# beast-dev/beast-mcmc

Measured on NVIDIA H100. Metric: tree log-likelihood evals/sec, higher is better.
Workload: dtype f64

## Files before the change

beast-mcmc_b200/beagle.py:

```python
from __future__ import annotations

import ctypes as C
import os
from typing import Optional, Sequence

import numpy as np

NONE = -1
OPERATION_TUPLE_SIZE = 7
PARTITION_OPERATION_TUPLE_SIZE = 9

_HERE = os.path.dirname(os.path.abspath(__file__))
_LIB = None


class BeagleException(RuntimeError):
    def __init__(self, functionName: str, errCode: int):
        super().__init__(f"BEAGLE function, {functionName}, returned error code {errCode}")
        self.functionName = functionName
        self.errCode = errCode


class BeagleErrorCode:
    NO_ERROR = 0
    GENERAL_ERROR = -1
    OUT_OF_MEMORY_ERROR = -2
    UNIDENTIFIED_EXCEPTION_ERROR = -3
    UNINITIALIZED_INSTANCE_ERROR = -4
    OUT_OF_RANGE_ERROR = -5
    NO_RESOURCE_ERROR = -6
    NO_IMPLEMENTATION_ERROR = -7
    FLOATING_POINT_ERROR = -8


class BeagleFlag:
    PRECISION_SINGLE = 1 << 0
    PRECISION_DOUBLE = 1 << 1
    COMPUTATION_SYNCH = 1 << 2
    COMPUTATION_ASYNCH = 1 << 3
    EIGEN_REAL = 1 << 4
    EIGEN_COMPLEX = 1 << 5
    SCALING_MANUAL = 1 << 6
    SCALING_AUTO = 1 << 7
    SCALING_ALWAYS = 1 << 8
    SCALERS_RAW = 1 << 9
    SCALERS_LOG = 1 << 10
    VECTOR_SSE = 1 << 11
    VECTOR_NONE = 1 << 12
    THREADING_OPENMP = 1 << 13
    THREADING_NONE = 1 << 14
    PROCESSOR_CPU = 1 << 15
    PROCESSOR_GPU = 1 << 16
    SCALING_DYNAMIC = 1 << 19
    FRAMEWORK_CUDA = 1 << 22
    FRAMEWORK_OPENCL = 1 << 23
    FRAMEWORK_CPU = 1 << 27
    PARALLELOPS_STREAMS = 1 << 28
    PARALLELOPS_GRID = 1 << 29
    THREADING_CPP = 1 << 30
    PREORDER_TRANSPOSE_AUTO = 1 << 31
    VECTOR_TENSOR = 1 << 33


class _InstanceDetailsStruct(C.Structure):
    _fields_ = [("resourceNumber", C.c_int), ("resourceName", C.c_char_p), ("implName", C.c_char_p),
                ("implDescription", C.c_char_p), ("flags", C.c_long)]


class _ResourceStruct(C.Structure):
    _fields_ = [("name", C.c_char_p), ("description", C.c_char_p), ("supportFlags", C.c_long),
                ("requiredFlags", C.c_long)]


class _ResourceListStruct(C.Structure):
    _fields_ = [("list", C.POINTER(_ResourceStruct)), ("length", C.c_int)]


class InstanceDetails:
    def __init__(self, resourceNumber=0, flags=0, resourceName="", implementationName=""):
        self.resourceNumber = resourceNumber
        self.flags = flags
        self.resourceName = resourceName
        self.implementationName = implementationName

    def getFlags(self):
        return self.flags

    def getResourceNumber(self):
        return self.resourceNumber


class ResourceDetails:
    def __init__(self, number, name, description, flags):
        self.number, self.name, self.description, self.flags = number, name, description, flags


_I = C.c_int
_IP = C.POINTER(C.c_int)
_DP = C.POINTER(C.c_double)
_L = C.c_long

_SIGNATURES = {
    "beagleGetVersion": ([], C.c_char_p),
    "beagleGetCitation": ([], C.c_char_p),
    "beagleGetResourceList": ([], C.POINTER(_ResourceListStruct)),
    "beagleGetBenchmarkedResourceList": ([_I, _I, _I, _I, _I, _IP, _I, _L, _L, _I, _I, _I, _L], C.c_void_p),
    "beagleCreateInstance": ([_I] * 9 + [_IP, _I, _L, _L, C.POINTER(_InstanceDetailsStruct)], _I),
    "beagleFinalizeInstance": ([_I], _I),
    "beagleFinalize": ([], _I),
    "beagleSetCPUThreadCount": ([_I, _I], _I),
    "beagleSetTipStates": ([_I, _I, _IP], _I),
    "beagleGetTipStates": ([_I, _I, _IP], _I),
    "beagleSetTipPartials": ([_I, _I, _DP], _I),
    "beagleSetPartials": ([_I, _I, _DP], _I),
    "beagleGetPartials": ([_I, _I, _I, _DP], _I),
    "beagleSetEigenDecomposition": ([_I, _I, _DP, _DP, _DP], _I),
    "beagleSetStateFrequencies": ([_I, _I, _DP], _I),
    "beagleSetCategoryWeights": ([_I, _I, _DP], _I),
    "beagleSetCategoryRates": ([_I, _DP], _I),
    "beagleSetCategoryRatesWithIndex": ([_I, _I, _DP], _I),
    "beagleSetPatternWeights": ([_I, _DP], _I),
    "beagleSetPatternPartitions": ([_I, _I, _IP], _I),
    "beagleUpdateTransitionMatrices": ([_I, _I, _IP, _IP, _IP, _DP, _I], _I),
    "beagleUpdateTransitionMatricesWithMultipleModels": ([_I, _IP, _IP, _IP, _IP, _IP, _DP, _I], _I),
    "beagleSetTransitionMatrix": ([_I, _I, _DP, C.c_double], _I),
    "beagleGetTransitionMatrix": ([_I, _I, _DP], _I),
    "beagleSetDifferentialMatrix": ([_I, _I, _DP], _I),
    "beagleConvolveTransitionMatrices": ([_I, _IP, _IP, _IP, _I], _I),
    "beagleAddTransitionMatrices": ([_I, _IP, _IP, _IP, _I], _I),
    "beagleTransposeTransitionMatrices": ([_I, _IP, _IP, _I], _I),
    "beagleUpdatePartials": ([_I, _IP, _I, _I], _I),
    "beagleUpdatePartialsByPartition": ([_I, _IP, _I], _I),
    "beagleWaitForPartials": ([_I, _IP, _I], _I),
    "beagleUpdatePrePartials": ([_I, _IP, _I, _I], _I),
    "beagleUpdatePrePartialsByPartition": ([_I, _IP, _I], _I),
    "beagleAccumulateScaleFactors": ([_I, _IP, _I, _I], _I),
    "beagleAccumulateScaleFactorsByPartition": ([_I, _IP, _I, _I, _I], _I),
    "beagleRemoveScaleFactors": ([_I, _IP, _I, _I], _I),
    "beagleRemoveScaleFactorsByPartition": ([_I, _IP, _I, _I, _I], _I),
    "beagleResetScaleFactors": ([_I, _I], _I),
    "beagleResetScaleFactorsByPartition": ([_I, _I, _I], _I),
    "beagleCopyScaleFactors": ([_I, _I, _I], _I),
    "beagleGetScaleFactors": ([_I, _I, _DP], _I),
    "beagleGetLogScaleFactors": ([_I, _I, _DP], _I),
    "beagleCalculateRootLogLikelihoods": ([_I, _IP, _IP, _IP, _IP, _I, _DP], _I),
    "beagleCalculateRootLogLikelihoodsByPartition": ([_I, _IP, _IP, _IP, _IP, _IP, _I, _I, _DP, _DP], _I),
    "beagleGetSiteLogLikelihoods": ([_I, _DP], _I),
    "beagleCalculateEdgeDerivatives": ([_I, _IP, _IP, _IP, _IP, _I, _DP, _DP, _DP], _I),
    "beagleCalculateCrossProductDerivative": ([_I, _IP, _IP, _IP, _IP, _DP, _I, _DP, _DP], _I),
    "b200SetKernelTiming": ([_I, _I], _I),
    "b200GetKernelTiming": ([_I, _I, _DP, C.POINTER(C.c_long)], _I),
    "b200CompressSitePatterns": ([_I, _I, _I, _IP, _DP, _IP, _IP, _DP, _IP], _I),
    "b200GetSourceHash": ([], C.c_char_p),
    "b200GetFusedLaunches": ([_I], _L),
    "b200RootLogLikelihoodsByPartitionDevice": ([_I, _IP, _IP, _IP, _IP, _IP, _I, C.POINTER(C.c_void_p), C.POINTER(C.c_void_p)], _I),
    "b200SetShardDevices": ([_IP, _I], _I),
    "b200ExchangeConnectLocal": ([_IP, _I], _I),
    "b200ExchangeCreate": ([_I, _I, _I, C.c_void_p], _I),
    "b200ExchangeConnect": ([_I, C.c_void_p], _I),
    "b200HostAlloc": ([_L], C.c_void_p),
    "b200HostFree": ([C.c_void_p], None),
    "b200DebugPlan": ([_I if False else _IP, _I, _I, _I, _I, _I, _I, _I, _IP, _IP, _IP, _IP], _I),
    "b200RootLogLikelihoodDevice": ([_I, _I, _I, _I, _I, C.POINTER(C.c_void_p), C.POINTER(C.c_void_p)], _I),
}


def exported_symbols():
    return list(_SIGNATURES.keys())


def load_library(path: Optional[str] = None):
    global _LIB
    if _LIB is not None and path is None:
        return _LIB
    path = path or os.environ.get("B200_BEAGLE_LIBRARY") or os.path.join(_HERE, "csrc", "libhmsbeagle.so")
    if not os.path.exists(path):
        raise FileNotFoundError(
            f"{path} not found: build it with `python -c 'import __graft_entry__ as g; g.build()'`; "
            "there is no CPU fallback for the product path")
    lib = C.CDLL(path)
    for name, (argtypes, restype) in _SIGNATURES.items():
        fn = getattr(lib, name)
        fn.argtypes = argtypes
        fn.restype = restype
    _LIB = lib
    return lib


def _ip(a):
    if a is None:
        return None
    a = np.ascontiguousarray(a, dtype=np.int32)
    return a, a.ctypes.data_as(_IP)


def _dp(a):
    a = np.ascontiguousarray(a, dtype=np.float64)
    return a, a.ctypes.data_as(_DP)


class Beagle:
    OPERATION_TUPLE_SIZE = OPERATION_TUPLE_SIZE
    PARTITION_OPERATION_TUPLE_SIZE = PARTITION_OPERATION_TUPLE_SIZE
    NONE = NONE


class BeagleJNIImpl(Beagle):

    def __init__(self, tipCount, partialsBufferCount, compactBufferCount, stateCount, patternCount,
                 eigenBufferCount, matrixBufferCount, categoryCount, scaleBufferCount,
                 resourceList: Optional[Sequence[int]], preferenceFlags: int, requirementFlags: int):
        self._lib = load_library()
        det = _InstanceDetailsStruct()
        rl = _ip(resourceList) if resourceList is not None else None
        inst = self._lib.beagleCreateInstance(tipCount, partialsBufferCount, compactBufferCount, stateCount,
                                              patternCount, eigenBufferCount, matrixBufferCount, categoryCount,
                                              scaleBufferCount, rl[1] if rl else None,
                                              len(resourceList) if resourceList is not None else 0,
                                              preferenceFlags, requirementFlags, C.byref(det))
        if inst < 0:
            raise BeagleException("create", inst)
        self.instance = inst
        self.patternCount = patternCount
        self.details = InstanceDetails(det.resourceNumber, det.flags,
                                       (det.resourceName or b"").decode(), (det.implName or b"").decode())

    def _check(self, name, rc):
        if rc != 0:
            raise BeagleException(name, rc)

    def getDetails(self):
        return self.details

    def finalize(self):
        if self.instance >= 0:
            rc = self._lib.beagleFinalizeInstance(self.instance)
            self.instance = -1
            self._check("finalize", rc)

    def setCPUThreadCount(self, threadCount):
        self._check("setCPUThreadCount", self._lib.beagleSetCPUThreadCount(self.instance, threadCount))

    def setPatternWeights(self, patternWeights):
        self._check("setPatternWeights", self._lib.beagleSetPatternWeights(self.instance, _dp(patternWeights)[1]))

    def setPatternPartitions(self, partitionCount, patternPartitions):
        self._check("setPatternPartitions",
                    self._lib.beagleSetPatternPartitions(self.instance, partitionCount, _ip(patternPartitions)[1]))

    def setTipStates(self, tipIndex, states):
        self._check("setTipStates", self._lib.beagleSetTipStates(self.instance, tipIndex, _ip(states)[1]))

    def getTipStates(self, tipIndex, states):
        self._check("getTipStates", self._lib.beagleGetTipStates(self.instance, tipIndex, states.ctypes.data_as(_IP)))

    def setTipPartials(self, tipIndex, partials):
        self._check("setTipPartials", self._lib.beagleSetTipPartials(self.instance, tipIndex, _dp(partials)[1]))

    def setPartials(self, bufferIndex, partials):
        self._check("setPartials", self._lib.beagleSetPartials(self.instance, bufferIndex, _dp(partials)[1]))

    def getPartials(self, bufferIndex, scaleIndex, outPartials):
        assert outPartials.dtype == np.float64 and outPartials.flags.c_contiguous
        self._check("getPartials", self._lib.beagleGetPartials(self.instance, bufferIndex, scaleIndex,
                                                               outPartials.ctypes.data_as(_DP)))

    def getLogScaleFactors(self, scaleIndex, outFactors):
        self._check("getLogScaleFactors", self._lib.beagleGetLogScaleFactors(self.instance, scaleIndex,
                                                                             outFactors.ctypes.data_as(_DP)))

    def getScaleFactors(self, scaleIndex, outFactors):
        self._check("getScaleFactors", self._lib.beagleGetScaleFactors(self.instance, scaleIndex,
                                                                       outFactors.ctypes.data_as(_DP)))

    def setEigenDecomposition(self, eigenIndex, eigenVectors, inverseEigenValues, eigenValues):
        self._check("setEigenDecomposition",
                    self._lib.beagleSetEigenDecomposition(self.instance, eigenIndex, _dp(eigenVectors)[1],
                                                          _dp(inverseEigenValues)[1], _dp(eigenValues)[1]))

    def setStateFrequencies(self, stateFrequenciesIndex, stateFrequencies):
        self._check("setStateFrequencies",
                    self._lib.beagleSetStateFrequencies(self.instance, stateFrequenciesIndex, _dp(stateFrequencies)[1]))

    def setCategoryWeights(self, categoryWeightsIndex, categoryWeights):
        self._check("setCategoryWeights",
                    self._lib.beagleSetCategoryWeights(self.instance, categoryWeightsIndex, _dp(categoryWeights)[1]))

    def setCategoryRates(self, inCategoryRates):
        self._check("setCategoryRates", self._lib.beagleSetCategoryRates(self.instance, _dp(inCategoryRates)[1]))

    def setCategoryRatesWithIndex(self, categoryRatesIndex, inCategoryRates):
        self._check("setCategoryRatesWithIndex",
                    self._lib.beagleSetCategoryRatesWithIndex(self.instance, categoryRatesIndex, _dp(inCategoryRates)[1]))

    def setTransitionMatrix(self, matrixIndex, inMatrix, paddedValue=0.0):
        self._check("setTransitionMatrix",
                    self._lib.beagleSetTransitionMatrix(self.instance, matrixIndex, _dp(inMatrix)[1], paddedValue))

    def getTransitionMatrix(self, matrixIndex, outMatrix):
        self._check("getTransitionMatrix",
                    self._lib.beagleGetTransitionMatrix(self.instance, matrixIndex, outMatrix.ctypes.data_as(_DP)))

    def updateTransitionMatrices(self, eigenIndex, probabilityIndices, firstDerivativeIndices,
                                 secondDerivativeIndices, edgeLengths, count):
        d1 = _ip(firstDerivativeIndices)
        d2 = _ip(secondDerivativeIndices)
        self._check("updateTransitionMatrices",
                    self._lib.beagleUpdateTransitionMatrices(self.instance, eigenIndex, _ip(probabilityIndices)[1],
                                                             d1[1] if d1 else None, d2[1] if d2 else None,
                                                             _dp(edgeLengths)[1], count))

    def updateTransitionMatricesWithMultipleModels(self, eigenIndices, categoryRateIndices, probabilityIndices,
                                                   firstDerivativeIndices, secondDerivativeIndices, edgeLengths, count):
        d1 = _ip(firstDerivativeIndices)
        d2 = _ip(secondDerivativeIndices)
# ... 161 lines not shown
```

beast-mcmc_b200/csrc/api.cu:

```cuda
#include "../../include/libhmsbeagle_b200.h"
#include "engine.h"
#include "multi.h"

#include <algorithm>
#include <atomic>
#include <chrono>
#include <cmath>
#include <cstdio>
#include <cstdlib>
#include <cstring>
#include <string>
#include <unordered_map>

using namespace b200;

namespace {

std::mutex gMutex;
std::vector<Instance*> gInstances;

const long kSupportedFlags =
    BEAGLE_FLAG_PRECISION_DOUBLE | BEAGLE_FLAG_PRECISION_SINGLE | BEAGLE_FLAG_COMPUTATION_SYNCH | BEAGLE_FLAG_EIGEN_REAL |
    BEAGLE_FLAG_EIGEN_COMPLEX | BEAGLE_FLAG_SCALING_MANUAL | BEAGLE_FLAG_SCALING_DYNAMIC |
    BEAGLE_FLAG_SCALERS_RAW | BEAGLE_FLAG_SCALERS_LOG | BEAGLE_FLAG_VECTOR_NONE | BEAGLE_FLAG_THREADING_NONE |
// ... 206 lines not shown
        plan.order.resize(n);
        for (int k = 0; k < n; ++k) plan.order[k] = k;
        plan.subs.assign(1, Sub{0, n, 0, 0});
        plan.phaseStart = {0, 1};
    };
    if (!allowReorder || n < 2) { single(); return; }
    std::vector<int> writer(nBuffers, -1);
    for (int k = 0; k < n; ++k) {
        if (writer[ops[k].dest] >= 0) { single(); return; }
        writer[ops[k].dest] = k;
    }
    std::vector<int> ch0(n, -1), ch1(n, -1), parent(n, -1);
    for (int k = 0; k < n; ++k) {
        const int a = writer[ops[k].c1], b = writer[ops[k].c2];
        if (a >= 0) { if (a >= k || parent[a] >= 0) { single(); return; } ch0[k] = a; parent[a] = k; }
        if (b >= 0 && ops[k].c2 != ops[k].c1) { if (b >= k || parent[b] >= 0) { single(); return; } ch1[k] = b; parent[b] = k; }
        if (ops[k].dest == ops[k].c1 || ops[k].dest == ops[k].c2) { single(); return; }
    }
    std::vector<char> alive(n, 1);
    std::vector<int> size(n), need(n);
    std::vector<std::pair<int, int>> stack;
    plan.order.clear(); plan.order.reserve(n);
    plan.subs.clear(); plan.phaseStart.assign(1, 0);
    int remaining = n;
    while (remaining > 0) {
        const int T = fixedT > 0 ? fixedT : (remaining <= smallRemainder ? remaining : std::max(minT, (remaining + wantSubs - 1) / wantSubs));
        for (int k = 0; k < n; ++k) {
            if (!alive[k]) continue;
            const int a = (ch0[k] >= 0 && alive[ch0[k]]) ? ch0[k] : -1;
            const int b = (ch1[k] >= 0 && alive[ch1[k]]) ? ch1[k] : -1;
            size[k] = 1 + (a >= 0 ? size[a] : 0) + (b >= 0 ? size[b] : 0);
            int na = a >= 0 ? need[a] : 0, nb = b >= 0 ? need[b] : 0;
            if (na < nb) std::swap(na, nb);
            need[k] = std::max(1, std::max(na, nb + (nb > 0 ? 1 : 0)));
        }
        for (int r = 0; r < n; ++r) {
            if (!alive[r] || size[r] > T) continue;
            if (parent[r] >= 0 && size[parent[r]] <= T) continue;
            const int begin = (int)plan.order.size();
            stack.push_back({r, 0});
            while (!stack.empty()) {
                auto [k, stageNo] = stack.back();
                stack.pop_back();
                if (stageNo == 1) { plan.order.push_back(k); continue; }
                stack.push_back({k, 1});
                const int a = (ch0[k] >= 0 && alive[ch0[k]]) ? ch0[k] : -1;
                const int b = (ch1[k] >= 0 && alive[ch1[k]]) ? ch1[k] : -1;
                const int na = a >= 0 ? need[a] : -1, nb = b >= 0 ? need[b] : -1;
                if (na >= nb) { if (b >= 0) stack.push_back({b, 0}); if (a >= 0) stack.push_back({a, 0}); }
                else          { if (a >= 0) stack.push_back({a, 0}); if (b >= 0) stack.push_back({b, 0}); }
            }
            plan.subs.push_back(Sub{begin, (int)plan.order.size(), 0, 0});
        }
        for (int q = plan.subs[plan.phaseStart.back()].begin; q < (int)plan.order.size(); ++q) alive[plan.order[q]] = 0;
        std::stable_sort(plan.subs.begin() + plan.phaseStart.back(), plan.subs.end(),
                         [](const Sub& a, const Sub& b) { return (a.end - a.begin) > (b.end - b.begin); });
        remaining = n - (int)plan.order.size();
        plan.phaseStart.push_back((int)plan.subs.size());
    }
}

void planLevels(const std::vector<HostOp>& ops, int nBuffers, Plan& plan) {
    const int n = (int)ops.size();
    std::vector<int> writer(nBuffers, -1), level(n, 0);
    bool hazard = false;
    for (int k = 0; k < n; ++k) { if (writer[ops[k].dest] >= 0) hazard = true; writer[ops[k].dest] = k; }
    int maxLevel = 0;
    for (int k = 0; k < n && !hazard; ++k) {
        for (int src : {ops[k].c1, ops[k].c2}) {
            const int w = writer[src];
            if (w < 0) continue;
            if (w >= k) { hazard = true; break; }
            level[k] = std::max(level[k], level[w] + 1);
        }
        maxLevel = std::max(maxLevel, level[k]);
    }
    plan.order.resize(n);
    for (int k = 0; k < n; ++k) plan.order[k] = k;
    plan.subs.clear();
    if (hazard) { plan.subs.assign(1, Sub{0, n, 0, 0}); plan.phaseStart = {0, 1}; return; }
    std::stable_sort(plan.order.begin(), plan.order.end(), [&](int a, int b) { return level[a] < level[b]; });
    plan.phaseStart.assign(1, 0);
    for (int pos = 0; pos < n; ++pos) {
        if (pos > 0 && level[plan.order[pos]] != level[plan.order[pos - 1]]) plan.phaseStart.push_back((int)plan.subs.size());
        plan.subs.push_back(Sub{pos, pos + 1, 0, 0});
    }
    plan.phaseStart.push_back((int)plan.subs.size());
}

void planPreorderPhases(const std::vector<HostOp>& ops, int nBuffers, int fixedT, int wantSubs, int minT,
                        int smallRemainder, Plan& plan) {
    const int n = (int)ops.size();
    std::vector<int> writer(nBuffers, -1), parent(n, -1);
    bool ok = n >= 2;
    for (int k = 0; k < n && ok; ++k) { ok = writer[ops[k].dest] < 0; writer[ops[k].dest] = k; }
    for (int k = 0; k < n && ok; ++k) {
        const int a = writer[ops[k].c1];
        ok = writer[ops[k].c2] < 0 && (a < 0 || a < k) && ops[k].dest != ops[k].c1 && ops[k].dest != ops[k].c2;
        parent[k] = a;
    }
    if (!ok) { planLevels(ops, nBuffers, plan); return; }
    std::vector<std::vector<int>> kids(n);
    for (int k = 0; k < n; ++k) if (parent[k] >= 0) kids[parent[k]].push_back(k);
    std::vector<char> alive(n, 1);
    std::vector<int> size(n), stack;
    std::vector<std::vector<int>> phases;
    int remaining = n;
    while (remaining > 0) {
        const int T = fixedT > 0 ? fixedT : (remaining <= smallRemainder ? remaining : std::max(minT, (remaining + wantSubs - 1) / wantSubs));
        for (int k = n - 1; k >= 0; --k) {
            if (!alive[k]) continue;
            size[k] = 1;
            for (int c : kids[k]) if (alive[c]) size[k] += size[c];
        }
        std::vector<int> roots;
        for (int r = 0; r < n; ++r)
            if (alive[r] && size[r] <= T && !(parent[r] >= 0 && alive[parent[r]] && size[parent[r]] <= T)) roots.push_back(r);
        for (int r : roots) {
            stack.assign(1, r);
            while (!stack.empty()) {
                const int k = stack.back(); stack.pop_back();
                if (!alive[k]) continue;
                alive[k] = 0; --remaining;
                for (int c : kids[k]) if (alive[c]) stack.push_back(c);
            }
        }
        phases.push_back(std::move(roots));
    }
    std::vector<int> phaseOf(n, -1), rootOf(n, -1);
    for (int ph = 0; ph < (int)phases.size(); ++ph)
        for (int r : phases[ph]) { phaseOf[r] = ph; rootOf[r] = r; }
    for (int k = 0; k < n; ++k)
        if (rootOf[k] < 0) { rootOf[k] = rootOf[parent[k]]; phaseOf[k] = phaseOf[parent[k]]; }
    plan.order.clear(); plan.order.reserve(n);
    plan.subs.clear(); plan.phaseStart.assign(1, 0);
    for (int ph = (int)phases.size() - 1; ph >= 0; --ph) {
        for (int r : phases[ph]) {
            const int begin = (int)plan.order.size();
            stack.assign(1, r);
            while (!stack.empty()) {
                const int k = stack.back(); stack.pop_back();
                plan.order.push_back(k);
                for (int q = (int)kids[k].size() - 1; q >= 0; --q)
                    if (rootOf[kids[k][q]] == r) stack.push_back(kids[k][q]);
            }
            plan.subs.push_back(Sub{begin, (int)plan.order.size(), 0, 0});
        }
        std::stable_sort(plan.subs.begin() + plan.phaseStart.back(), plan.subs.end(),
                         [](const Sub& a, const Sub& b) { return (a.end - a.begin) > (b.end - b.begin); });
        plan.phaseStart.push_back((int)plan.subs.size());
    }
}

cudaError_t launchPlan(Instance* in, const void* dOps, const void* dSubs, const std::vector<int>& phaseStart,
                       const std::vector<int>& phaseDepth, bool fourPath, int maxWindow, bool preOrder, int eigenSlot = -1,
                       bool aligned = false, const void* dSnap = nullptr, int nSnap = 0, const void* dVirtTips = nullptr) {
    const bool virt = dVirtTips != nullptr;
    cudaError_t e = cudaSuccess;
    if (nSnap > 0) {
        TimedScope ts(in, T_PARTIALS);
        e = launchCherrySnapshot(in, static_cast<const int4*>(dSnap), nSnap);
    }
    for (size_t ph = 0; ph + 1 < phaseStart.size() && e == cudaSuccess; ++ph) {
        const int s0 = phaseStart[ph], s1 = phaseStart[ph + 1];
        if (s1 <= s0) continue;
        TimedScope ts(in, T_PARTIALS);
        if (fourPath && eigenSlot >= 0 && !preOrder && (ph >= phaseDepth.size() || phaseDepth[ph] == 0)) {
            e = launchWalk4E(in, static_cast<const Op4*>(dOps), static_cast<const int4*>(dSubs) + s0, s1 - s0, maxWindow,
                             aligned, in->hEigen.data() + (size_t)eigenSlot * 36, static_cast<const int4*>(dVirtTips));
            continue;
        }
        if (virt) return cudaErrorInvalidValue;
        e = fourPath ? launchWalk4(in, static_cast<const Op4*>(dOps), static_cast<const int4*>(dSubs) + s0, s1 - s0,
                                   ph < phaseDepth.size() ? phaseDepth[ph] : 0, maxWindow, preOrder)
                     : launchWalkGeneric(in, static_cast<const DevOp*>(dOps), static_cast<const int4*>(dSubs) + s0, s1 - s0,
                                         maxWindow, preOrder);
    }
    return e;
}

cudaError_t accumulateInList(Instance* in, const std::vector<CumGroup>& groups) {
    for (const CumGroup& g : groups) {
        int* dIdx = static_cast<int*>(stage(in, g.indices.data(), sizeof(int) * g.indices.size()));
        if (dIdx == nullptr) return cudaErrorMemoryAllocation;
        cudaError_t e = launchScaleAccumulate(in, dIdx, (int)g.indices.size(), in->dScale + (size_t)g.cum * in->Ppad, 1.0,
                                              g.pBegin, g.pEnd);
        if (e != cudaSuccess) return e;
        in->scaleIsLog[g.cum] = 1;
    }
    return cudaSuccess;
}

void noteScaleWrites(Instance* in, const std::vector<HostOp>& hops) {
    for (const HostOp& o : hops) if (o.sw >= 0) in->scaleIsLog[o.sw] = in->logScalers ? 1 : 0;
}


cudaError_t storeCherries(Instance* in, const int* bufs, int count) {
    if (in->cherryTip1.empty()) return cudaSuccess;
    std::vector<int4> items;
    for (int k = 0; k < count; ++k) {
        const int b = bufs[k];
        if (!validRange(b, in->nBuffers) || in->cherryTip1[b] < 0 || in->cherryStored[b]) continue;
        items.push_back(make_int4(in->slotOf[b], b, in->cherryTip1[b], in->cherryTip2[b]));
        in->cherryStored[b] = 1;
    }
    if (items.empty()) return cudaSuccess;
    const int4* dItems = static_cast<const int4*>(stage(in, items.data(), sizeof(int4) * items.size()));
    cudaError_t e = cudaErrorMemoryAllocation;
    if (dItems != nullptr) {
        TimedScope ts(in, T_PARTIALS);
        e = launchCherryStore(in, dItems, (int)items.size());
    }
    if (e != cudaSuccess) for (const int4& it : items) in->cherryStored[it.y] = 0;
    return e;
}

cudaError_t storeExternal(Instance* in, const std::vector<CherryRef>& external) {
    std::vector<int> bufs;
    for (const CherryRef& x : external) if (x.tip1 < 0) bufs.push_back(x.buf);
    return storeCherries(in, bufs.data(), (int)bufs.size());
}

cudaError_t settleCherriesOf(Instance* in, int t) {
    std::vector<int> deps;
    for (int b = 0; b < (int)in->cherryTip1.size(); ++b)
        if (in->cherryTip1[b] >= 0 && (in->cherryTip1[b] == t || in->cherryTip2[b] == t)) deps.push_back(b);
    const cudaError_t e = storeCherries(in, deps.data(), (int)deps.size());
    if (e == cudaSuccess) for (int b : deps) in->cherryTip1[b] = -1;
    return e;
}

void noteCherryWrites(Instance* in, const std::vector<HostOp>& hops, const std::vector<CherryRef>& cherries) {
    if (in->cherryTip1.empty()) return;
    for (const HostOp& o : hops) in->cherryTip1[o.dest] = -1;
    for (const CherryRef& c : cherries) {
        in->cherryTip1[c.buf] = c.tip1; in->cherryTip2[c.buf] = c.tip2; in->cherryStored[c.buf] = 0;
    }
}

int prepareOps(Instance* in, const std::vector<HostOp>& hops, bool byPartition) {
    for (const HostOp& o : hops) {
        if (!validRange(o.dest, in->nBuffers) || !validRange(o.c1, in->nBuffers) ||
            !validRange(o.c2, in->nBuffers) || !validRange(o.m1, in->nMatrices) ||
            !validRange(o.m2, in->nMatrices))
            return BEAGLE_ERROR_OUT_OF_RANGE;
        if (o.sw != BEAGLE_OP_NONE && !validRange(o.sw, in->nScale)) return BEAGLE_ERROR_OUT_OF_RANGE;
        if (o.sr != BEAGLE_OP_NONE && !validRange(o.sr, in->nScale)) return BEAGLE_ERROR_OUT_OF_RANGE;
        if (o.cum != BEAGLE_OP_NONE && !validRange(o.cum, in->nScale)) return BEAGLE_ERROR_OUT_OF_RANGE;
        if (byPartition && !validRange(o.part, in->partitionCount)) return BEAGLE_ERROR_OUT_OF_RANGE;
    }
    {
        std::vector<char> written(in->nBuffers, 0);
        for (const HostOp& o : hops) written[o.dest] = 1;
        auto holdsData = [&](int b) { return written[b] || in->partials[b] != nullptr || in->states32[b] != nullptr; };
        for (const HostOp& o : hops) {
            if (!holdsData(o.c1) || !holdsData(o.c2)) return BEAGLE_ERROR_OUT_OF_RANGE;
            if (o.kind == 1 && !written[o.c1] && in->states32[o.c1] != nullptr) return BEAGLE_ERROR_OUT_OF_RANGE;
        }
    }
    for (const HostOp& o : hops) {
        if (ensurePartials(in, o.dest) == nullptr) return BEAGLE_ERROR_OUT_OF_MEMORY;
        if (in->states32[o.dest] != nullptr) in->bufferEpoch++;
        in->states8[o.dest] = nullptr;
        in->states32[o.dest] = nullptr;
    }
    return BEAGLE_SUCCESS;
}

int eigenFormSlot(const Instance* in, const std::vector<HostOp>& hops) {
    if (!in->eigenWalk || in->matCP == 0 || in->walkVariant != 0 || hops.empty() || hops[0].kind == 1) return -1;
    const int E = in->matEigen[hops[0].m1];
    if (E < 0 || !in->eigenReal[E]) return -1;
    const unsigned gen = in->eigenGen[E];
    for (const HostOp& o : hops)
        if (in->matEigen[o.m1] != E || in->matEigen[o.m2] != E || in->matEigenGen[o.m1] != gen || in->matEigenGen[o.m2] != gen)
            return -1;
    return E;
}

int planAndLaunch(Instance* in, const std::vector<HostOp>& hops, bool byPartition) {
    const int n = (int)hops.size();
    if (n == 0) return BEAGLE_SUCCESS;
    static_assert(sizeof(HostOp) == 10 * sizeof(int), "HostOp is compared bytewise");
    if (in->planCacheSize > 0) {
        for (CachedPlan& cp : in->planCache) {
            if (cp.dBlock == nullptr || cp.n != n || cp.byPartition != byPartition || cp.epoch != in->bufferEpoch ||
                memcmp(cp.key.data(), hops.data(), sizeof(HostOp) * (size_t)n) != 0)
                continue;
            const int eigenSlot = cp.fourPath ? eigenFormSlot(in, hops) : -1;
            bool stale = cp.readsVirtual && eigenSlot < 0;
            for (const CherryRef& x : cp.external)
                stale = stale || (x.tip1 >= 0 && (in->cherryTip1[x.buf] != x.tip1 || in->cherryTip2[x.buf] != x.tip2));
            if (stale) { cp.dropGraph(); cp.n = -1; continue; }
            CUDA_OK(storeExternal(in, cp.external));
            cp.lastUse = ++in->planClock;
            cp.hits++;
            const unsigned eigenGenNow = eigenSlot >= 0 ? in->eigenGen[eigenSlot] : 0u;
            const void* dSnap = static_cast<char*>(cp.dBlock) + cp.snapOffset;
            const int nSnap = (int)cp.cherries.size();
            const void* dTips = cp.readsVirtual ? static_cast<char*>(cp.dBlock) + cp.tipsOffset : nullptr;
            if (cp.graphExec != nullptr && (cp.graphEigen != eigenSlot || cp.graphEigenGen != eigenGenNow)) {
                if (cp.graphAllEigen && eigenSlot >= 0 && cp.graphEigen == eigenSlot &&
                    updateWalk4EGraph(cp.graphExec, cp.graphKernelNodes, in->hEigen.data() + (size_t)eigenSlot * 36) == cudaSuccess) {
                    cp.graphEigenGen = eigenGenNow;
                } else {
                    cudaGetLastError();
                    cp.dropGraph();
                    cp.hits = 1;
                    if (++cp.graphInvalidations >= 4) cp.graphFailed = true;
                }
            }
            int launches = nSnap > 0;
            for (size_t ph = 0; ph + 1 < cp.phaseStart.size(); ++ph) launches += cp.phaseStart[ph + 1] > cp.phaseStart[ph];
            if (in->useGraphs && launches >= 2 && cp.cumGroups.empty()) {
                if (cp.graphExec == nullptr && !cp.graphFailed && cp.hits >= 2 && !in->timing &&
                    cudaStreamBeginCapture(in->stream, cudaStreamCaptureModeThreadLocal) == cudaSuccess) {
                    const cudaError_t e1 = launchPlan(in, cp.dBlock, static_cast<char*>(cp.dBlock) + cp.subsOffset, cp.phaseStart,
                                                      cp.phaseDepth, cp.fourPath, cp.maxWindow, cp.preOrder, eigenSlot,
                                                      !cp.byPartition, dSnap, nSnap, dTips);
                    cp.graphEigen = eigenSlot;
                    cp.graphEigenGen = eigenGenNow;
                    cudaGraph_t g = nullptr;
                    const cudaError_t e2 = cudaStreamEndCapture(in->stream, &g);
                    if (e1 != cudaSuccess || e2 != cudaSuccess || g == nullptr ||
                        cudaGraphInstantiate(&cp.graphExec, g, 0) != cudaSuccess) {
                        cp.graphExec = nullptr;
                        cp.graphFailed = true;
                        if (g) cudaGraphDestroy(g);
                    } else {
                        cp.graph = g;
                        cp.graphKernelNodes.clear();
                        cp.graphAllEigen = cp.fourPath && eigenSlot >= 0 && !cp.preOrder;
                        for (int dpt : cp.phaseDepth) cp.graphAllEigen = cp.graphAllEigen && dpt == 0;
                        size_t nn = 0;
                        if (cudaGraphGetNodes(g, nullptr, &nn) == cudaSuccess && nn > 0) {
                            std::vector<cudaGraphNode_t> nodes(nn);
                            cudaGraphNodeType ty;
                            if (cudaGraphGetNodes(g, nodes.data(), &nn) == cudaSuccess)
                                for (size_t q = 0; q < nn; ++q)
                                    if (cudaGraphNodeGetType(nodes[q], &ty) == cudaSuccess && ty == cudaGraphNodeTypeKernel)
                                        cp.graphKernelNodes.push_back(nodes[q]);
                        }
                        if (cp.graphKernelNodes.empty()) cp.graphAllEigen = false;
                    }
                    if (getenv("B200_BEAGLE_DEBUG"))
                        fprintf(stderr, "[b200-beagle] graph %s: %d launches\n", cp.graphExec ? "captured" : "capture failed",
                                launches);
                    cudaGetLastError();
                }
                if (cp.graphExec != nullptr) {
                    TimedScope ts(in, T_PARTIALS, launches);
                    CUDA_OK(cudaGraphLaunch(cp.graphExec, in->stream));
                    noteScaleWrites(in, hops);
                    noteCherryWrites(in, hops, cp.cherries);
                    return BEAGLE_SUCCESS;
                }
            }
            CUDA_OK(launchPlan(in, cp.dBlock, static_cast<char*>(cp.dBlock) + cp.subsOffset, cp.phaseStart, cp.phaseDepth,
                               cp.fourPath, cp.maxWindow, cp.preOrder, eigenSlot, !cp.byPartition, dSnap, nSnap,
                               dTips));
            CUDA_OK(accumulateInList(in, cp.cumGroups));
            noteScaleWrites(in, hops);
            noteCherryWrites(in, hops, cp.cherries);
            return BEAGLE_SUCCESS;
        }
    }
    {
        const int rcPrepare = prepareOps(in, hops, byPartition);
        if (rcPrepare != BEAGLE_SUCCESS) return rcPrepare;
    }
    const bool fourState = in->matCP > 0;
    const bool preOrder = hops[0].kind == 1;
    const int eigenSlot = fourState ? eigenFormSlot(in, hops) : -1;
    std::vector<char> written(in->nBuffers, 0);
    std::vector<int> firstWrite(in->nBuffers, n);
    for (int k = n - 1; k >= 0; --k) { written[hops[k].dest] = 1; firstWrite[hops[k].dest] = k; }
    std::vector<CherryRef> cherries;
    std::vector<int4> snap;
    std::vector<HostOp> kept;
    bool readsVirtual = false;
    if (!in->cherryTip1.empty() && !byPartition && !preOrder && eigenSlot >= 0 && !in->stackTail) {
        std::vector<int> writes(in->nBuffers, 0), firstRead(in->nBuffers, n);
        for (int k = 0; k < n; ++k) {
            writes[hops[k].dest]++;
            firstRead[hops[k].c1] = std::min(firstRead[hops[k].c1], k);
            firstRead[hops[k].c2] = std::min(firstRead[hops[k].c2], k);
        }
        for (int k = 0; k < n; ++k) {
            const HostOp& o = hops[k];
            if (in->states8[o.c1] != nullptr && in->states8[o.c2] != nullptr && o.sw == BEAGLE_OP_NONE &&
                o.sr == BEAGLE_OP_NONE && o.cum == BEAGLE_OP_NONE && writes[o.dest] == 1 && firstRead[o.dest] > k) {
                cherries.push_back(CherryRef{o.dest, o.c1, o.c2});
                snap.push_back(make_int4(o.dest, o.m1, o.m2, 0));
            } else {
                kept.push_back(o);
            }
        }
        if (kept.empty()) { cherries.clear(); snap.clear(); }
        readsVirtual = !cherries.empty();
        for (const HostOp& o : hops)
            for (int c : {o.c1, o.c2})
                readsVirtual = readsVirtual || (!written[c] && in->states32[c] == nullptr && in->cherryTip1[c] >= 0);
    }
    Plan plan;
    int maxWindow = in->Ppad;
    const int patsPerWarp = !fourState ? 16 : (in->walkVariant == 2 ? 8 * in->tensorR : (32 / in->matCP) * in->walkR);
    const int warpsPerSM = fourState ? 32 : 12;
    auto wantSubsFor = [&](int window) {
        const int warpsPerSub = std::max(1, (window + patsPerWarp - 1) / patsPerWarp);
        const int over = in->phaseOversub > 0 ? in->phaseOversub : (warpsPerSub >= 32 ? 1 : 2);
        return std::max(1, over * ((in->smCount * warpsPerSM + warpsPerSub - 1) / warpsPerSub));
    };
    if (!byPartition && !preOrder) {
        planPhases(cherries.empty() ? hops : kept, in->nBuffers, in->reorder != 0, in->phaseT, wantSubsFor(in->Ppad),
                   in->phaseTmin, in->phaseSmall, plan);
        bool served = true;
        for (size_t ph = 0; readsVirtual && ph + 1 < plan.phaseStart.size(); ++ph) {
            const int nSubs = plan.phaseStart[ph + 1] - plan.phaseStart[ph];
            served = served && (nSubs == 0 || walk4pServes(in, nSubs, in->Ppad));
        }
        if (!served) {
            readsVirtual = false;
            if (!cherries.empty()) {
                cherries.clear(); snap.clear(); kept.clear();
                planPhases(hops, in->nBuffers, in->reorder != 0, in->phaseT, wantSubsFor(in->Ppad), in->phaseTmin,
                           in->phaseSmall, plan);
            }
        }
        for (Sub& sb : plan.subs) { sb.pBase = 0; sb.pLimit = in->Ppad; }
    }
    const std::vector<HostOp>& L = cherries.empty() ? hops : kept;
    const int nL = (int)L.size();
    std::vector<int> vt1(readsVirtual ? in->nBuffers : 0, -1), vt2(readsVirtual ? in->nBuffers : 0, -1);
    for (const CherryRef& c : cherries) { vt1[c.buf] = c.tip1; vt2[c.buf] = c.tip2; }
    std::vector<CherryRef> external;
    {
        std::vector<char> seen(in->nBuffers, 0);
        for (int k = 0; k < n; ++k)
            for (int c : {hops[k].c1, hops[k].c2}) {
                if (firstWrite[c] < k || in->states32[c] != nullptr || seen[c]) continue;
                seen[c] = 1;
                const bool virt = readsVirtual && !written[c] && in->cherryTip1[c] >= 0;
                external.push_back(CherryRef{c, virt ? in->cherryTip1[c] : -1, virt ? in->cherryTip2[c] : -1});
                if (virt) { vt1[c] = in->cherryTip1[c]; vt2[c] = in->cherryTip2[c]; }
            }
    }
    CUDA_OK(storeExternal(in, external));
    {
        if (!byPartition) {
            if (preOrder) {
                if (in->prePhases) planPreorderPhases(hops, in->nBuffers, in->phaseT, wantSubsFor(in->Ppad), in->phaseTmin, in->phaseSmall, plan);
                else planLevels(hops, in->nBuffers, plan);
                for (Sub& sb : plan.subs) { sb.pBase = 0; sb.pLimit = in->Ppad; }
            }
        } else {
            std::vector<std::vector<int>> members(in->partitionCount);
            for (int k = 0; k < n; ++k) members[hops[k].part].push_back(k);
            std::vector<Plan> plans;
            std::vector<int> base;
            maxWindow = 1;
            for (int part = 0; part < in->partitionCount; ++part) {
                if (members[part].empty()) continue;
                std::vector<HostOp> sub(members[part].size());
                for (size_t q = 0; q < sub.size(); ++q) sub[q] = hops[members[part][q]];
                Plan pl;
                const int window = in->partEnd[part] - in->partBegin[part];
                if (sub[0].kind == 1 && in->prePhases) planPreorderPhases(sub, in->nBuffers, in->phaseT, wantSubsFor(std::max(1, window)), in->phaseTmin, in->phaseSmall, pl);
                else if (sub[0].kind == 1) planLevels(sub, in->nBuffers, pl);
                else planPhases(sub, in->nBuffers, in->reorder != 0, in->phaseT, wantSubsFor(std::max(1, window)), in->phaseTmin, in->phaseSmall, pl);
                base.push_back((int)plan.order.size());
                for (int idx : pl.order) plan.order.push_back(members[part][idx]);
                for (Sub& sb : pl.subs) {
                    sb.begin += base.back(); sb.end += base.back();
                    sb.pBase = in->partBegin[part]; sb.pLimit = in->partEnd[part];
                }
                maxWindow = std::max(maxWindow, window);
                plans.push_back(std::move(pl));
            }
            plan.phaseStart.assign(1, 0);
            for (size_t ph = 0;; ++ph) {
                bool any = false;
                for (const Plan& pl : plans) {
                    if (ph + 1 >= pl.phaseStart.size()) continue;
                    any = true;
                    for (int q = pl.phaseStart[ph]; q < pl.phaseStart[ph + 1]; ++q) plan.subs.push_back(pl.subs[q]);
                }
                if (!any) break;
                plan.phaseStart.push_back((int)plan.subs.size());
            }
        }
    }
    const std::vector<int>& order = plan.order;

    const bool stackEverywhere = fourState && in->walkVariant == 1 && !preOrder;
    const bool stackThin = fourState && in->walkVariant == 0 && in->stackTail && !preOrder;
    const int maxDepth = (stackEverywhere || stackThin) ? in->stackDepthMax : 0;
    const int nPhases = (int)plan.phaseStart.size() - 1;
    std::vector<char> subStack(plan.subs.size(), 0);
    std::vector<int> phaseDepth(std::max(nPhases, 1), 0), phaseOfSub(plan.subs.size(), 0);
    if (maxDepth > 0) {
        const int patsPerWarpS = (32 / in->matCP) * in->walkR;
        for (int ph = 0; ph < nPhases; ++ph) {
            long warps = 0;
            for (int q = plan.phaseStart[ph]; q < plan.phaseStart[ph + 1]; ++q) {
                warps += (plan.subs[q].pLimit - plan.subs[q].pBase + patsPerWarpS - 1) / patsPerWarpS;
                phaseOfSub[q] = ph;
            }
            const bool thin = warps < (long)in->smCount * 8;
            for (int q = plan.phaseStart[ph]; q < plan.phaseStart[ph + 1]; ++q) subStack[q] = stackEverywhere || thin;
        }
    }
    std::vector<int> lastReadOfProd(maxDepth > 0 ? nL : 0, -1);
    std::vector<int> subOfPos(nL, 0);
    for (int sIdx = 0; sIdx < (int)plan.subs.size(); ++sIdx)
        for (int q = plan.subs[sIdx].begin; q < plan.subs[sIdx].end; ++q) subOfPos[q] = sIdx;
    if (maxDepth > 0) {
        std::vector<int> lastRead(in->nBuffers, -1);
        for (size_t sIdx = 0; sIdx < plan.subs.size(); ++sIdx) {
            if (!subStack[sIdx]) continue;
            const Sub& sb = plan.subs[sIdx];
            for (int pos = sb.end - 1; pos >= sb.begin; --pos) {
                const HostOp& o = L[order[pos]];
                lastReadOfProd[pos] = lastRead[o.dest];
                lastRead[o.dest] = -1;
                if (lastRead[o.c1] < 0) lastRead[o.c1] = pos;
                if (lastRead[o.c2] < 0) lastRead[o.c2] = pos;
            }
            for (int pos = sb.begin; pos < sb.end; ++pos) {
                const HostOp& o = L[order[pos]];
                lastRead[o.dest] = lastRead[o.c1] = lastRead[o.c2] = -1;
            }
        }
    }
    std::vector<int> slotOf(maxDepth > 0 ? in->nBuffers : 0, -1), slotFreeAt(maxDepth > 0 ? in->nBuffers : 0, -1);
    std::vector<int> freeSlots;
    int depthUsed = 0, depthThisSub = 0, curSub = -1;

    const bool fourPath = in->matCP > 0;
    std::vector<CumGroup> cumGroups;
    std::vector<DevOp> dops(fourPath ? 0 : nL);
    std::vector<Op4> ops4(fourPath ? nL : 0);
    std::vector<int4> virtTips(readsVirtual ? nL : 0);
    for (int pos = 0; pos < nL; ++pos) {
        const HostOp& o = L[order[pos]];
        const bool t1 = in->states32[o.c1] != nullptr;
        const bool t2 = in->states32[o.c2] != nullptr;
        int srcSlot1 = -1, srcSlot2 = -1, dstSlot = -1;
        if (maxDepth > 0 && subOfPos[pos] != curSub) {
            curSub = subOfPos[pos];
            freeSlots.clear();
            depthThisSub = 0;
        }
        if (maxDepth > 0 && subStack[subOfPos[pos]]) {
            auto take = [&](int buf, bool isTip) -> int {
                if (isTip) return -1;
                const int slot = slotOf[buf];
                if (slot >= 0 && slotFreeAt[buf] == pos) { freeSlots.push_back(slot); slotOf[buf] = -1; }
                return slot;
            };
            srcSlot1 = take(o.c1, t1);
            srcSlot2 = (o.c2 == o.c1) ? srcSlot1 : take(o.c2, t2);
            if (slotOf[o.dest] >= 0) { freeSlots.push_back(slotOf[o.dest]); slotOf[o.dest] = -1; }
            if (lastReadOfProd[pos] > pos) {
                int slot = -1;
                if (!freeSlots.empty()) { slot = freeSlots.back(); freeSlots.pop_back(); }
                else if (depthThisSub < maxDepth) {
                    slot = depthThisSub++;
                    depthUsed = std::max(depthUsed, depthThisSub);
                    phaseDepth[phaseOfSub[subOfPos[pos]]] = std::max(phaseDepth[phaseOfSub[subOfPos[pos]]], depthThisSub);
                }
                if (slot >= 0) { slotOf[o.dest] = slot; slotFreeAt[o.dest] = lastReadOfProd[pos]; dstSlot = slot; }
            }
        }
        const int pBegin = byPartition ? in->partBegin[o.part] : 0;
        const int pEnd = byPartition ? in->partEnd[o.part] : in->P;
        if (o.cum >= 0 && o.sw >= 0) {
            CumGroup* grp = nullptr;
            for (CumGroup& g : cumGroups) if (g.cum == o.cum && g.pBegin == pBegin && g.pEnd == pEnd) { grp = &g; break; }
            if (grp == nullptr) { cumGroups.push_back(CumGroup{o.cum, pBegin, pEnd, {}}); grp = &cumGroups.back(); }
            grp->indices.push_back(o.sw);
        }
        const int cum = -1;
        if (fourPath) {
            Op4& d = ops4[pos];
            const bool v1 = readsVirtual && !t1 && vt1[o.c1] >= 0, v2 = readsVirtual && !t2 && vt1[o.c2] >= 0;
            d.dest = in->slotOf[o.dest];
            d.c1 = t1 ? -(o.c1 + 1) : v1 ? o.c1 : in->slotOf[o.c1];
            d.c2 = t2 ? -(o.c2 + 1) : v2 ? o.c2 : in->slotOf[o.c2];
            d.m1 = o.m1; d.m2 = o.m2; d.sw = o.sw; d.sr = o.sr; d.cum = cum;
            d.pBegin = pBegin; d.pEnd = pEnd;
            d.slots = (unsigned)(srcSlot1 & 0xFF) | ((unsigned)(srcSlot2 & 0xFF) << 8) | ((unsigned)(dstSlot & 0xFF) << 16);
            d.pad_ = o.kind | (v1 ? 4 : 0) | (v2 ? 8 : 0);
            d.pfA = d.pfB = 0; d.pfM1 = d.pfM2 = -1;
            if (readsVirtual)
                virtTips[pos] = make_int4(v1 ? vt1[o.c1] : 0, v1 ? vt2[o.c1] : 0, v2 ? vt1[o.c2] : 0, v2 ? vt2[o.c2] : 0);
            if (in->forward && !(maxDepth > 0 && subStack[subOfPos[pos]]) && pos > plan.subs[subOfPos[pos]].begin) {
                const Op4& pv = ops4[pos - 1];
                if (pv.pBegin == d.pBegin && pv.pEnd == d.pEnd) {
                    if (!t1 && !v1 && d.c1 == pv.dest) d.pad_ |= 2;
                    else if (!preOrder && !t2 && !v2 && d.c2 == pv.dest) {
                        std::swap(d.c1, d.c2); std::swap(d.m1, d.m2);
                        if (readsVirtual) { int4& t = virtTips[pos]; t = make_int4(t.z, t.w, t.x, t.y); }
                        d.pad_ = (d.pad_ & ~12) | (v1 ? 8 : 0) | 2;
                    }
                }
            }
        } else {
            DevOp& d = dops[pos];
            memset(&d, 0, sizeof d);
            d.dest = reinterpret_cast<double*>(in->partials[o.dest]);
            d.c1 = t1 ? nullptr : reinterpret_cast<const double*>(in->partials[o.c1]);
            d.c2 = t2 ? nullptr : reinterpret_cast<const double*>(in->partials[o.c2]);
            d.s1 = t1 ? (const void*)in->states32[o.c1] : nullptr;
            d.s2 = t2 ? (const void*)in->states32[o.c2] : nullptr;
            d.m1 = in->dMat + (size_t)o.m1 * in->matStride;
            d.m2 = in->dMat + (size_t)o.m2 * in->matStride;
            d.scaleWrite = o.sw >= 0 ? in->dScale + (size_t)o.sw * in->Ppad : nullptr;
            d.scaleRead = o.sr >= 0 ? in->dScale + (size_t)o.sr * in->Ppad : nullptr;
            d.cumScale = cum >= 0 ? in->dScale + (size_t)cum * in->Ppad : nullptr;
            d.pBegin = pBegin; d.pEnd = pEnd;
            d.srcSlot1 = d.srcSlot2 = d.dstSlot = -1;
            d.pad_ = o.kind;
            if (in->forward && !preOrder && pos > plan.subs[subOfPos[pos]].begin) {
                const DevOp& pv = dops[pos - 1];
                if (pv.pBegin == d.pBegin && pv.pEnd == d.pEnd) {
                    if (d.c1 != nullptr && d.c1 == pv.dest) d.pad_ |= 2;
                    else if (d.c2 != nullptr && d.c2 == pv.dest) {
                        std::swap(d.c1, d.c2); std::swap(d.s1, d.s2); std::swap(d.m1, d.m2); d.pad_ |= 2;
                    }
                }
            }
        }
    }
    if (fourPath && in->lookahead && (!preOrder || in->lookaheadPre)) {
        std::vector<char> thick(plan.subs.size(), 0);
        const long perSub = (maxWindow + (32 / in->matCP) * in->walkR - 1) / ((32 / in->matCP) * in->walkR);
        for (int ph = 0; ph < nPhases; ++ph) {
            const bool t = (long)(plan.phaseStart[ph + 1] - plan.phaseStart[ph]) * perSub >= (long)in->smCount * 8;
            for (int q = plan.phaseStart[ph]; q < plan.phaseStart[ph + 1]; ++q) thick[q] = t;
        }
        for (size_t sIdx = 0; sIdx < plan.subs.size(); ++sIdx) {
            if ((maxDepth > 0 && subStack[sIdx]) || (!thick[sIdx] && in->lookahead < 2)) continue;
            for (int pos = plan.subs[sIdx].begin; pos + 1 < plan.subs[sIdx].end; ++pos) {
                Op4& d = ops4[pos];
                const Op4& nx = ops4[pos + 1];
                auto enc = [&](int child, bool fromRegisters, bool virt) -> int {
                    if (fromRegisters || virt) return 0;
                    if (child < 0) return ((-child - 1) << 1) | 1;
                    return child == d.dest ? 0 : ((child + 1) << 1);
                };
                d.pfA = enc(nx.c1, (nx.pad_ & 2) != 0, (nx.pad_ & 4) != 0);
                d.pfB = enc(nx.c2, false, (nx.pad_ & 8) != 0);
                if (d.pfA == 0) { d.pfA = d.pfB; d.pfB = 0; }
                d.pfM1 = nx.m1; d.pfM2 = nx.m2;
            }
        }
    }
    if (fourPath && getenv("B200_BEAGLE_DEBUG")) {
        int fwd = 0, internal = 0;
        for (const Op4& d : ops4) { fwd += (d.pad_ & 2) != 0; internal += (d.c1 >= 0) + (d.c2 >= 0); }
        fprintf(stderr, "[b200-beagle] plan: %d ops (%zu virtual cherries), %zu subtrees, %d phases, %d internal children, "
                "%d forwarded in registers\n", nL, cherries.size(), plan.subs.size(), nPhases, internal, fwd);
    }
    const size_t opBytes = (fourPath ? sizeof(Op4) : sizeof(DevOp)) * (size_t)nL;
    const size_t subBytes = sizeof(Sub) * plan.subs.size();
    const size_t snapBytes = sizeof(int4) * snap.size();
    const size_t subsOffset = (opBytes + 255) & ~size_t(255);
    const size_t snapOffset = subsOffset + ((subBytes + 255) & ~size_t(255));
    const size_t tipsBytes = sizeof(int4) * virtTips.size();
    const size_t tipsOffset = snapOffset + ((snapBytes + 255) & ~size_t(255));
    const size_t blockBytes = tipsOffset + tipsBytes;
    std::vector<char> hBlock(blockBytes, 0);
    memcpy(hBlock.data(), fourPath ? (const void*)ops4.data() : (const void*)dops.data(), opBytes);
    memcpy(hBlock.data() + subsOffset, plan.subs.data(), subBytes);
    if (snapBytes) memcpy(hBlock.data() + snapOffset, snap.data(), snapBytes);
    if (tipsBytes) memcpy(hBlock.data() + tipsOffset, virtTips.data(), tipsBytes);
    void* dOps = stage(in, hBlock.data(), blockBytes);
    void* tmp = nullptr;
    if (dOps == nullptr) {
        CUDA_OK(cudaMalloc(&tmp, blockBytes));
        dOps = tmp;
        cudaError_t ce = cudaMemcpyAsync(dOps, hBlock.data(), blockBytes, cudaMemcpyHostToDevice, in->stream);
        if (ce == cudaSuccess) ce = cudaStreamSynchronize(in->stream);
        if (ce != cudaSuccess) { cudaFree(tmp); CUDA_OK(ce); }
    }
    void* dSubs = static_cast<char*>(dOps) + subsOffset;
    std::vector<int> depths(plan.phaseStart.size(), 0);
    for (size_t ph = 0; ph + 1 < plan.phaseStart.size(); ++ph) depths[ph] = (maxDepth > 0 && ph < phaseDepth.size()) ? phaseDepth[ph] : 0;
    cudaError_t e = launchPlan(in, dOps, dSubs, plan.phaseStart, depths, fourPath, maxWindow, preOrder, eigenSlot, !byPartition,
                               static_cast<char*>(dOps) + snapOffset, (int)snap.size(),
                               readsVirtual ? static_cast<char*>(dOps) + tipsOffset : nullptr);
    if (e == cudaSuccess) e = accumulateInList(in, cumGroups);
    noteScaleWrites(in, hops);
    if (e == cudaSuccess) noteCherryWrites(in, hops, cherries);
    if (e == cudaSuccess && tmp == nullptr && in->planCacheSize > 0) {
        if ((int)in->planCache.size() < in->planCacheSize) in->planCache.emplace_back();
        CachedPlan* slot = nullptr;
        for (CachedPlan& cp : in->planCache) {
            if (cp.dBlock == nullptr || cp.n < 0) { slot = &cp; break; }
            if (slot == nullptr || cp.lastUse < slot->lastUse) slot = &cp;
        }
        slot->dropGraph();
        slot->hits = 0;
        slot->graphFailed = false;
        slot->graphInvalidations = 0;
        if (slot->capacity < blockBytes) {
            if (slot->dBlock) cudaFree(slot->dBlock);
            slot->dBlock = nullptr; slot->capacity = 0;
            if (cudaMalloc(&slot->dBlock, blockBytes) == cudaSuccess) slot->capacity = blockBytes; else cudaGetLastError();
        }
        if (slot->dBlock != nullptr &&
            cudaMemcpyAsync(slot->dBlock, dOps, blockBytes, cudaMemcpyDeviceToDevice, in->stream) == cudaSuccess) {
            slot->key = hops; slot->n = n; slot->byPartition = byPartition; slot->epoch = in->bufferEpoch;
            slot->subsOffset = subsOffset; slot->snapOffset = snapOffset; slot->tipsOffset = tipsOffset;
            slot->cherries = cherries; slot->external = external; slot->readsVirtual = readsVirtual;
            slot->phaseStart = plan.phaseStart; slot->phaseDepth = depths;
            slot->fourPath = fourPath; slot->maxWindow = maxWindow; slot->preOrder = preOrder;
            slot->lastUse = ++in->planClock;
            slot->cumGroups = cumGroups;
            slot->graphFailed = !cumGroups.empty();
        } else if (slot->dBlock != nullptr) {
            slot->n = -1;
        }
    }
    if (tmp != nullptr) { cudaStreamSynchronize(in->stream); cudaFree(tmp); }
    CUDA_OK(e);
    return BEAGLE_SUCCESS;
}

}

namespace b200 {
Instance* instanceById(int id) { return getInstance(id); }
}

extern "C" {

#ifndef B200_SOURCE_HASH
#define B200_SOURCE_HASH "unhashed"
#endif
const char* beagleGetVersion(void) { return "4.0.1-b200+" B200_SOURCE_HASH; }
const char* b200GetSourceHash(void) { return B200_SOURCE_HASH; }

const char* beagleGetCitation(void) {
    return "H100-native tree-likelihood engine exposing the BEAGLE API.\n"
           "API after: Ayres et al. (2019) BEAGLE 3. Syst Biol 68:1052-1061.";
}

BeagleResourceList* beagleGetResourceList(void) {
    std::call_once(gResourceOnce, buildResources);
    return &gResourceList;
}

BeagleBenchmarkedResourceList* beagleGetBenchmarkedResourceList(
    int tipCount, int compactBufferCount, int stateCount, int patternCount, int categoryCount, int* resourceList,
    int resourceCount, long preferenceFlags, long requirementFlags, int eigenModelCount, int partitionCount,
    int calculateDerivatives, long benchmarkFlags);

int beagleCreateInstance(int tipCount, int partialsBufferCount, int compactBufferCount, int stateCount,
                         int patternCount, int eigenBufferCount, int matrixBufferCount, int categoryCount,
                         int scaleBufferCount, int* resourceList, int resourceCount, long preferenceFlags,
                         long requirementFlags, BeagleInstanceDetails* returnInfo) {
    if (tipCount < 0 || partialsBufferCount < 0 || compactBufferCount < 0 || stateCount < 2 ||
        patternCount < 1 || eigenBufferCount < 0 || matrixBufferCount < 0 || categoryCount < 1 ||
        scaleBufferCount < 0 || stateCount > 255)
        return BEAGLE_ERROR_OUT_OF_RANGE;
    if (requirementFlags & ~kSupportedFlags) return BEAGLE_ERROR_NO_RESOURCE;
    const bool singleFits = stateCount <= 4 && categoryCount <= 8;
    if (requirementFlags & BEAGLE_FLAG_PRECISION_SINGLE) {
        if (!singleFits || (requirementFlags & BEAGLE_FLAG_PRECISION_DOUBLE)) return BEAGLE_ERROR_NO_RESOURCE;
    }
    const bool single = singleFits && ((requirementFlags & BEAGLE_FLAG_PRECISION_SINGLE) ||
                                       ((preferenceFlags & BEAGLE_FLAG_PRECISION_SINGLE) &&
                                        !((preferenceFlags | requirementFlags) & BEAGLE_FLAG_PRECISION_DOUBLE)));
    BeagleResourceList* rl = beagleGetResourceList();
    int resource = -1;
    if (resourceList == nullptr || resourceCount <= 0) {
        if (rl->length > 1) resource = 1;
    } else {
        for (int k = 0; k < resourceCount; ++k)
            if (resourceList[k] >= 1 && resourceList[k] < rl->length) { resource = resourceList[k]; break; }
    }
    if (resource < 1) return BEAGLE_ERROR_NO_RESOURCE;

    if (resource == gShardResource) {
        Instance* parent = new Instance();
        parent->resource = resource;
        parent->device = gShardDevices[0];
        parent->P = patternCount; parent->S = stateCount; parent->C = categoryCount; parent->tipCount = tipCount;
        const int g = (int)gShardDevices.size();
        const int rc = shardedCreate(parent, g, gShardDevices.data(), tipCount, partialsBufferCount, compactBufferCount,
                                     stateCount, patternCount, eigenBufferCount, matrixBufferCount, categoryCount,
                                     scaleBufferCount, preferenceFlags, requirementFlags, returnInfo);
        if (rc != BEAGLE_SUCCESS) { delete parent; return rc; }
        if (returnInfo != nullptr) {
            returnInfo->resourceNumber = resource;
            returnInfo->resourceName = rl->list[resource].name;
            parent->flags = returnInfo->flags;
        }
        std::lock_guard<std::mutex> lock(gMutex);
        int id = -1;
        for (size_t k = 0; k < gInstances.size(); ++k) if (gInstances[k] == nullptr) { id = (int)k; break; }
        if (id < 0) { gInstances.push_back(nullptr); id = (int)gInstances.size() - 1; }
        gInstances[id] = parent;
        parent->id = id;
        return id;
    }

    Instance* in = new Instance();
    in->device = resource - 1;
    in->resource = resource;
    if (cudaSetDevice(in->device) != cudaSuccess) { delete in; return BEAGLE_ERROR_NO_RESOURCE; }
    in->tipCount = tipCount; in->nPartials = partialsBufferCount; in->nCompact = compactBufferCount;
    in->S = stateCount; in->P = patternCount; in->nEigen = eigenBufferCount; in->nMatrices = matrixBufferCount;
    in->C = categoryCount; in->nScale = scaleBufferCount;
    in->Sp = stateCount <= 4 ? 4 : ((stateCount + 7) / 8) * 8;
    in->Ppad = ((patternCount + 31) / 32) * 32;
    in->nBuffers = partialsBufferCount + compactBufferCount;
    in->nSets = std::max(1, eigenBufferCount);
    in->single = single;
    in->complexEigen = (requirementFlags | preferenceFlags) & BEAGLE_FLAG_EIGEN_COMPLEX;
    in->logScalers = (requirementFlags | preferenceFlags) & BEAGLE_FLAG_SCALERS_LOG;
    in->flags = (single ? BEAGLE_FLAG_PRECISION_SINGLE : BEAGLE_FLAG_PRECISION_DOUBLE) | BEAGLE_FLAG_COMPUTATION_SYNCH |
                BEAGLE_FLAG_SCALING_MANUAL |
                BEAGLE_FLAG_VECTOR_NONE | BEAGLE_FLAG_THREADING_NONE | BEAGLE_FLAG_PROCESSOR_GPU |
                BEAGLE_FLAG_FRAMEWORK_CUDA | BEAGLE_FLAG_PARALLELOPS_GRID |
                (in->complexEigen ? BEAGLE_FLAG_EIGEN_COMPLEX : BEAGLE_FLAG_EIGEN_REAL) |
                (in->logScalers ? BEAGLE_FLAG_SCALERS_LOG : BEAGLE_FLAG_SCALERS_RAW);
    if ((requirementFlags | preferenceFlags) & BEAGLE_FLAG_PREORDER_TRANSPOSE_AUTO) in->flags |= BEAGLE_FLAG_PREORDER_TRANSPOSE_AUTO;
    if ((requirementFlags | preferenceFlags) & BEAGLE_FLAG_SCALING_DYNAMIC) {
        in->flags &= ~BEAGLE_FLAG_SCALING_MANUAL;
        in->flags |= BEAGLE_FLAG_SCALING_DYNAMIC;
    }
    in->partialsElems = (size_t)in->C * in->Ppad * in->Sp;
    if (in->Sp == 4 && in->C <= 32) {
        int cp = 1;
        while (cp < in->C) cp <<= 1;
        in->matCP = cp;
        in->matStride = (size_t)16 * cp + 52 * (size_t)in->C;
        in->matStride = (in->matStride + 3) & ~size_t(3);
    } else {
        in->matCP = 0;
        in->matStride = (size_t)in->C * in->Sp * (in->Sp + 2 * (size_t)(in->Sp + 4));
    }
    in->slotOf.assign(in->nBuffers, -1);
    in->partials.assign(in->nBuffers, nullptr);
    in->states8.assign(in->nBuffers, nullptr);
    in->states32.assign(in->nBuffers, nullptr);
    in->scaleIsLog.assign(std::max(1, in->nScale), in->logScalers ? 1 : 0);
    in->matEigen.assign(std::max(1, in->nMatrices), -1);
    in->matEigenGen.assign(std::max(1, in->nMatrices), 0u);
    in->eigenGen.assign(std::max(1, in->nEigen), 0u);
    in->eigenReal.assign(std::max(1, in->nEigen), 0);
    in->hEigen.assign((size_t)std::max(1, in->nEigen) * 36, 0.0);
    in->eigenWalk = envInt("B200_EIGEN_WALK", 1);
    in->tipMode = envInt("B200_TIP_MODE", 3);
    in->thinTipMode = envInt("B200_THIN_TIP_MODE", in->tipMode);
    in->virtualCherries = envInt("B200_VIRTUAL_CHERRIES", 1);
    in->walkBlock = 128;
    in->walkVariant = envInt("B200_WALK_VARIANT", 0);
    in->reorder = envInt("B200_REORDER", 1);
    in->forward = envInt("B200_FORWARD", 1);
    in->lookahead = envInt("B200_LOOKAHEAD", 1);
    in->useGraphs = envInt("B200_GRAPHS", 1);
    in->prePhases = envInt("B200_PRE_PHASES", 1);
    in->lookaheadPre = envInt("B200_LOOKAHEAD_PRE", 1);
    in->planCacheSize = std::max(0, std::min(16, envInt("B200_PLAN_CACHE", 4)));
    in->planCache.reserve(16);
    in->thinR1 = envInt("B200_THIN_R1", 1);
    in->stackTail = envInt("B200_STACK_TAIL", 0);
    in->phaseT = envInt("B200_PHASE_T", 0);
    in->phaseTmin = std::max(1, envInt("B200_PHASE_TMIN", 4));
    in->phaseSmall = envInt("B200_PHASE_SMALL", 24);
    in->phaseOversub = std::max(0, envInt("B200_PHASE_OVERSUB", 0));
    in->walkMinBlocks = envInt("B200_WALK_MINB", 4);
    in->walkMinBlocksSet = getenv("B200_WALK_MINB") != nullptr;
    in->tensorR = envInt("B200_TENSOR_R", 2) >= 4 ? 4 : 2;
    in->genericMma = envInt("B200_GENERIC_MMA", 1);
    in->mmaWarps = envInt("B200_MMA_WARPS", 4) == 8 ? 8 : 4;
    cudaDeviceProp prop;
    bool ok = cudaGetDeviceProperties(&prop, in->device) == cudaSuccess;
    if (ok) { in->smCount = prop.multiProcessorCount; in->maxSmemOptin = prop.sharedMemPerBlockOptin; }
    in->walkR = envInt("B200_WALK_R", 4);
    if (in->walkR != 1 && in->walkR != 2 && in->walkR != 4 && in->walkR != 8) in->walkR = 4;
    if (getenv("B200_WALK_R") == nullptr && in->matCP > 0) {
        const int G = 32 / in->matCP;
        while (in->walkR > 1 && (in->Ppad + G * in->walkR - 1) / (G * in->walkR) < in->smCount) in->walkR >>= 1;
    }
    in->stackDepthMax = std::min(64, std::max(0, envInt("B200_STACK_DEPTH", 12)));
    if (single) { in->walkVariant = 0; in->stackTail = 0; }

    ok = ok && cudaStreamCreateWithFlags(&in->stream, cudaStreamNonBlocking) == cudaSuccess;
    const size_t eigenStride = 2 * (size_t)in->S * in->S + 2 * in->S;
    const size_t matElems = (size_t)in->nMatrices * in->matStride;
    const int rootBlocks = (in->Ppad + 255) / 256;
    in->stageSize = size_t(8) << 20;
    auto alloc = [&](auto** p, size_t elems) {
        if (!ok) return;
        using T = std::remove_pointer_t<std::remove_pointer_t<decltype(p)>>;
        size_t bytes = std::max<size_t>(elems, 1) * sizeof(T);
        ok = cudaMalloc(reinterpret_cast<void**>(p), bytes) == cudaSuccess &&
             cudaMemsetAsync(*p, 0, bytes, in->stream) == cudaSuccess;
    };
    alloc(&in->dEigen, std::max(1, in->nEigen) * eigenStride);
    alloc(&in->dMat, matElems);
    if (in->matCP > 0) alloc(&in->dEvec, (size_t)in->nMatrices * in->matCP * 4);
    if (in->matCP > 0 && in->matCP <= 8 && in->virtualCherries) {
        alloc(&in->dRecipe, (size_t)in->nBuffers * 32 * in->matCP);
        in->cherryTip1.assign(in->nBuffers, -1);
        in->cherryTip2.assign(in->nBuffers, -1);
        in->cherryStored.assign(in->nBuffers, 0);
    }
    if (in->matCP > 0 && in->matCP <= 8) {
        alloc(&in->dIncSums, (size_t)in->Ppad / 4 + 8);
        alloc(&in->dIncCounter, 4);
        in->fuseSmall = envInt("B200_FUSE", 1);
        if (ok && in->fuseSmall) {
            if (cudaHostAlloc(reinterpret_cast<void**>(&in->hMapped), 64, cudaHostAllocMapped) == cudaSuccess &&
                cudaHostGetDevicePointer(reinterpret_cast<void**>(&in->dMapped), in->hMapped, 0) == cudaSuccess) {
                memset(in->hMapped, 0, 64);
            } else {
                cudaGetLastError();
                if (in->hMapped) cudaFreeHost(in->hMapped);
                in->hMapped = nullptr;
            }
        }
    }
    alloc(&in->dRates, (size_t)in->nSets * in->C);
    alloc(&in->dWeights, (size_t)in->nSets * in->C);
    alloc(&in->dFreqs, (size_t)in->nSets * in->Sp);
    alloc(&in->dScale, (size_t)in->nScale * in->Ppad);
    alloc(&in->dPatternWeights, in->Ppad);
    alloc(&in->dPatternPartitions, in->Ppad);
    alloc(&in->dSite, in->Ppad);
    alloc(&in->dBlockSums, rootBlocks);
    alloc(&in->dOut, 1024);
    alloc(&in->dCounter, 4);
    alloc(&in->dStage, in->stageSize);
    alloc(&in->states8Base, (size_t)std::max(1, in->tipCount) * in->Ppad);
    alloc(&in->states32Base, (size_t)std::max(1, in->tipCount) * in->Ppad);
    if (ok) {
        int want[2] = {in->nPartials, std::max(1, in->nPartials - std::min(in->nCompact, in->tipCount))};
        for (int attempt = 0; attempt < 2 && in->partialsBase == nullptr; ++attempt) {
            size_t bytes = (size_t)want[attempt] * in->partialsElems * in->elemBytes();
            if (cudaMalloc(reinterpret_cast<void**>(&in->partialsBase), bytes) == cudaSuccess) in->nSlots = want[attempt];
            else { cudaGetLastError(); in->partialsBase = nullptr; }
        }
        if (in->partialsBase == nullptr) { destroyInstance(in); return BEAGLE_ERROR_OUT_OF_MEMORY; }
    }
    ok = ok && cudaMallocHost(reinterpret_cast<void**>(&in->hStage), in->stageSize) == cudaSuccess;
    ok = ok && cudaMallocHost(reinterpret_cast<void**>(&in->hOut), 1024 * sizeof(double)) == cudaSuccess;
    if (ok) {
        in->hRates.assign((size_t)in->nSets * in->C, 1.0);
        in->hWeights.assign((size_t)in->nSets * in->C, 0.0);
        in->hFreqs.assign((size_t)in->nSets * 4, 0.0);
        std::vector<double> ones((size_t)std::max(in->nSets * in->C, in->Ppad), 1.0);
        ok = cudaMemcpyAsync(in->dRates, ones.data(), sizeof(double) * in->nSets * in->C, cudaMemcpyHostToDevice,
                             in->stream) == cudaSuccess;
        std::vector<double> w(in->Ppad, 0.0);
        std::fill(w.begin(), w.begin() + in->P, 1.0);
        ok = ok && cudaMemcpyAsync(in->dPatternWeights, w.data(), sizeof(double) * in->Ppad, cudaMemcpyHostToDevice,
                                   in->stream) == cudaSuccess;
        ok = ok && cudaStreamSynchronize(in->stream) == cudaSuccess;
    }
    if (!ok) {
        cudaError_t e = cudaGetLastError();
        destroyInstance(in);
        return e == cudaErrorMemoryAllocation ? BEAGLE_ERROR_OUT_OF_MEMORY : BEAGLE_ERROR_GENERAL;
    }
    in->partitionCount = 1;
    in->partBegin.assign(1, 0);
    in->partEnd.assign(1, in->P);
    {
        std::lock_guard<std::mutex> lock(gMutex);
        int id = -1;
        for (size_t k = 0; k < gInstances.size(); ++k) if (gInstances[k] == nullptr) { id = (int)k; break; }
        if (id < 0) { gInstances.push_back(nullptr); id = (int)gInstances.size() - 1; }
        gInstances[id] = in;
        in->id = id;
    }
    if (returnInfo != nullptr) {
        returnInfo->resourceNumber = resource;
        returnInfo->resourceName = rl->list[resource].name;
        returnInfo->implName = single ? gImplNameSingle : gImplName;
        returnInfo->implDescription = gImplDesc;
        returnInfo->flags = in->flags;
    }
    return in->id;
}

int beagleFinalizeInstance(int instance) {
    Instance* in = nullptr;
    {
        std::lock_guard<std::mutex> lock(gMutex);
        if (instance < 0 || instance >= (int)gInstances.size() || gInstances[instance] == nullptr)
            return BEAGLE_ERROR_UNINITIALIZED_INSTANCE;
        in = gInstances[instance];
        gInstances[instance] = nullptr;
    }
    destroyInstance(in);
    return BEAGLE_SUCCESS;
}

int beagleFinalize(void) {
    std::vector<Instance*> all;
    {
        std::lock_guard<std::mutex> lock(gMutex);
        all.swap(gInstances);
    }
    for (Instance* in : all) if (in) destroyInstance(in);
    return BEAGLE_SUCCESS;
}

int beagleSetCPUThreadCount(int instance, int) {
    SH(instance, BEAGLE_SUCCESS);
// ... 762 lines not shown
                                                 const int* categoryWeightsIndices,
                                                 const int* stateFrequenciesIndices,
                                                 const int* cumulativeScaleIndices, const int* partitionIndices,
                                                 int partitionCount, int count,
                                                 double* outSumLogLikelihoodByPartition, double* outSumLogLikelihood) {
    SH(instance, BEAGLE_ERROR_NO_IMPLEMENTATION);
    GET_INSTANCE(in, instance);
    if (count != 1) return BEAGLE_ERROR_NO_IMPLEMENTATION;
    int rc = rootByPartitionLaunch(in, bufferIndices, categoryWeightsIndices, stateFrequenciesIndices,
                                   cumulativeScaleIndices, partitionIndices, partitionCount);
    if (rc != BEAGLE_SUCCESS) return rc;
    const int extra = in->exchangeOn ? 2 : 0;
    CUDA_OK(cudaMemcpyAsync(in->hOut, in->dOut, sizeof(double) * (partitionCount + extra), cudaMemcpyDeviceToHost, in->stream));
    CUDA_OK(cudaStreamSynchronize(in->stream));
    double total = 0.0;
    for (int k = 0; k < partitionCount; ++k) { outSumLogLikelihoodByPartition[k] = in->hOut[k]; total += in->hOut[k]; }
    if (in->exchangeOn) total = in->hOut[partitionCount];
    *outSumLogLikelihood = total;
    return std::isnan(total) ? BEAGLE_ERROR_FLOATING_POINT : BEAGLE_SUCCESS;
}

int beagleGetSiteLogLikelihoods(int instance, double* outLogLikelihoods) {
    SH(instance, shGetPerPattern(sh, outLogLikelihoods, [&](int c, double* o) { return beagleGetSiteLogLikelihoods(c, o); }));
    GET_INSTANCE(in, instance);
    CUDA_OK(cudaMemcpyAsync(outLogLikelihoods, in->dSite, sizeof(double) * in->P, cudaMemcpyDeviceToHost, in->stream));
    CUDA_OK(cudaStreamSynchronize(in->stream));
    return BEAGLE_SUCCESS;
}

static cudaError_t ensureScratch(Instance* in, size_t doubles) {
    if (doubles <= in->scratchDoubles) return cudaSuccess;
    cudaError_t e = cudaStreamSynchronize(in->stream);
    if (e != cudaSuccess) return e;
    cudaFree(in->dScratch);
    in->dScratch = nullptr;
    in->scratchDoubles = 0;
    e = cudaMalloc(reinterpret_cast<void**>(&in->dScratch), doubles * sizeof(double));
    if (e == cudaSuccess) in->scratchDoubles = doubles;
    return e;
}

int beagleCalculateEdgeDerivatives(int instance, const int* postBufferIndices, const int* preBufferIndices,
                                   const int* derivativeMatrixIndices, const int* categoryWeightsIndices, int count,
                                   double* outDerivatives, double* outSumDerivatives, double* outSumSquaredDerivatives) {
    SH(instance, shEdgeDerivatives(sh, postBufferIndices, preBufferIndices, derivativeMatrixIndices, categoryWeightsIndices, count, outDerivatives, outSumDerivatives, outSumSquaredDerivatives));
    GET_INSTANCE(in, instance);
    if (count <= 0) return BEAGLE_SUCCESS;
    if (!validRange(categoryWeightsIndices[0], in->nSets)) return BEAGLE_ERROR_OUT_OF_RANGE;
    std::vector<EdgeRefT<void>> edges(count);
    for (int e = 0; e < count; ++e) {
        const int po = postBufferIndices[e], pr = preBufferIndices[e], dm = derivativeMatrixIndices[e];
        if (!validRange(po, in->nBuffers) || !validRange(pr, in->nBuffers) || !validRange(dm, in->nMatrices) ||
            in->partials[pr] == nullptr || (in->partials[po] == nullptr && in->states32[po] == nullptr))
            return BEAGLE_ERROR_OUT_OF_RANGE;
        edges[e].post = in->states32[po] != nullptr ? nullptr : in->partials[po];
        edges[e].states = in->states32[po];
        edges[e].pre = in->partials[pr];
        edges[e].D = in->dMat + (size_t)dm * in->matStride;
        edges[e].len = 0.0;
    }
    CUDA_OK(storeCherries(in, postBufferIndices, count));
    const size_t perEdge = outDerivatives != nullptr ? (size_t)in->P : 0;
    const size_t edgeDoubles = ((size_t)count * sizeof(EdgeRefT<void>) + 7) / 8;
    const size_t results = (size_t)count * (2 + perEdge);
    const size_t partials = edgeDerivativeWorkspace(in, count);
    CUDA_OK(ensureScratch(in, edgeDoubles + results + partials));
    EdgeRefT<void>* dEdges = reinterpret_cast<EdgeRefT<void>*>(in->dScratch);
    double* dOut = in->dScratch + edgeDoubles;
    CUDA_OK(cudaMemcpyAsync(dEdges, edges.data(), sizeof(EdgeRefT<void>) * count, cudaMemcpyHostToDevice, in->stream));
    {
        TimedScope ts(in, T_ROOT);
        CUDA_OK(launchEdgeDerivatives(in, dEdges, count, in->dWeights + (size_t)categoryWeightsIndices[0] * in->C,
                                      perEdge ? dOut + 2 * (size_t)count : nullptr, dOut, dOut + count,
                                      partials ? dOut + results : nullptr));
    }
    std::vector<double> host(results);
    CUDA_OK(cudaMemcpyAsync(host.data(), dOut, sizeof(double) * results, cudaMemcpyDeviceToHost, in->stream));
    CUDA_OK(cudaStreamSynchronize(in->stream));
    for (int k = 0; k < count; ++k) {
        if (outSumDerivatives) outSumDerivatives[k] = host[k];
        if (outSumSquaredDerivatives) outSumSquaredDerivatives[k] = host[count + k];
    }
    if (outDerivatives) memcpy(outDerivatives, host.data() + 2 * (size_t)count, sizeof(double) * (size_t)count * in->P);
    return BEAGLE_SUCCESS;
}

int beagleCalculateCrossProductDerivative(int instance, const int* postBufferIndices, const int* preBufferIndices,
                                          const int* categoryRatesIndices, const int* categoryWeightsIndices,
                                          const double* edgeLengths, int count, double* outSumDerivatives,
                                          double* outSumSquaredDerivatives) {
    SH(instance, shCrossProducts(sh, postBufferIndices, preBufferIndices, categoryRatesIndices, categoryWeightsIndices, edgeLengths, count, outSumDerivatives, outSumSquaredDerivatives));
    GET_INSTANCE(in, instance);
    if (outSumSquaredDerivatives != nullptr) return BEAGLE_ERROR_NO_IMPLEMENTATION;
    if (count <= 0) return BEAGLE_SUCCESS;
    if (outSumDerivatives == nullptr || edgeLengths == nullptr) return BEAGLE_ERROR_OUT_OF_RANGE;
    if (!validRange(categoryRatesIndices[0], in->nSets) || !validRange(categoryWeightsIndices[0], in->nSets))
        return BEAGLE_ERROR_OUT_OF_RANGE;
    const size_t n = (size_t)in->S * in->S;
    const size_t edgeDoubles = ((size_t)count * sizeof(EdgeRefT<void>) + 7) / 8;
    const size_t need = edgeDoubles + ((size_t)crossProductBlocks(in, count) + 1) * n;
    CUDA_OK(ensureScratch(in, need));
    std::vector<EdgeRefT<void>> edges(count);
    for (int e = 0; e < count; ++e) {
        const int po = postBufferIndices[e], pr = preBufferIndices[e];
        if (!validRange(po, in->nBuffers) || !validRange(pr, in->nBuffers) || in->partials[pr] == nullptr ||
            (in->partials[po] == nullptr && in->states32[po] == nullptr))
            return BEAGLE_ERROR_OUT_OF_RANGE;
        edges[e].post = in->states32[po] != nullptr ? nullptr : in->partials[po];
        edges[e].states = in->states32[po];
        edges[e].pre = in->partials[pr];
        edges[e].D = nullptr;
        edges[e].len = edgeLengths[e];
    }
    CUDA_OK(storeCherries(in, postBufferIndices, count));
    EdgeRefT<void>* dEdges = reinterpret_cast<EdgeRefT<void>*>(in->dScratch);
    double* work = in->dScratch + edgeDoubles;
    CUDA_OK(cudaMemcpyAsync(dEdges, edges.data(), sizeof(EdgeRefT<void>) * count, cudaMemcpyHostToDevice, in->stream));
    {
        TimedScope ts(in, T_ROOT);
        CUDA_OK(launchCrossProducts(in, dEdges, count, in->dRates + (size_t)categoryRatesIndices[0] * in->C,
                                    in->dWeights + (size_t)categoryWeightsIndices[0] * in->C, work));
    }
    std::vector<double> host(n);
    CUDA_OK(cudaMemcpyAsync(host.data(), work + (size_t)crossProductBlocks(in, count) * n, sizeof(double) * n,
                            cudaMemcpyDeviceToHost, in->stream));
    CUDA_OK(cudaStreamSynchronize(in->stream));
    for (size_t q = 0; q < n; ++q) outSumDerivatives[q] += host[q];
    return BEAGLE_SUCCESS;
}

int b200DebugPlan(const int* operations, int operationCount, int bufferCount, int fixedT, int wantSubs, int minT,
                  int smallRemainder, int preOrder, int* outOrder, int* outSubs, int* outPhaseStart, int* outCounts) {
    if (operationCount < 0 || bufferCount <= 0) return BEAGLE_ERROR_OUT_OF_RANGE;
    std::vector<HostOp> hops(operationCount);
    for (int k = 0; k < operationCount; ++k) {
        const int* o = operations + 7 * k;
        for (int f : {o[0], o[3], o[5]}) if (f < 0 || f >= bufferCount) return BEAGLE_ERROR_OUT_OF_RANGE;
        hops[k] = {o[0], o[1], o[2], o[3], o[4], o[5], o[6], 0, -1};
        hops[k].kind = preOrder ? 1 : 0;
    }
    Plan plan;
    if (operationCount == 0) { outCounts[0] = outCounts[1] = 0; return BEAGLE_SUCCESS; }
    if (preOrder == 2) planLevels(hops, bufferCount, plan);
    else if (preOrder) planPreorderPhases(hops, bufferCount, fixedT, std::max(1, wantSubs), std::max(1, minT), smallRemainder, plan);
    else planPhases(hops, bufferCount, true, fixedT, std::max(1, wantSubs), std::max(1, minT), smallRemainder, plan);
    for (int k = 0; k < operationCount; ++k) outOrder[k] = plan.order[k];
    for (size_t q = 0; q < plan.subs.size(); ++q) { outSubs[2 * q] = plan.subs[q].begin; outSubs[2 * q + 1] = plan.subs[q].end; }
    for (size_t q = 0; q < plan.phaseStart.size(); ++q) outPhaseStart[q] = plan.phaseStart[q];
    outCounts[0] = (int)plan.subs.size();
    outCounts[1] = (int)plan.phaseStart.size() - 1;
    return BEAGLE_SUCCESS;
}

int b200SetKernelTiming(int instance, int enable) {
    SH(instance, shBroadcast(sh, [&](int c) { return b200SetKernelTiming(c, enable); }));
    GET_INSTANCE(in, instance);
    CUDA_OK(cudaStreamSynchronize(in->stream));
    for (int c = 0; c < T_CLASSES; ++c) {
        for (auto& ev : in->timed[c]) { cudaEventDestroy(ev.first); cudaEventDestroy(ev.second); }
        in->timed[c].clear();
        in->timedMs[c] = 0.0;
        in->timedLaunches[c] = 0;
    }
    in->timing = enable != 0;
    return BEAGLE_SUCCESS;
}

int b200GetKernelTiming(int instance, int which, double* outMilliseconds, long* outLaunches) {
    GET_INSTANCE(in, instance);
    if (which < 0 || which >= T_CLASSES) return BEAGLE_ERROR_OUT_OF_RANGE;
    CUDA_OK(cudaStreamSynchronize(in->stream));
    for (auto& ev : in->timed[which]) {
        float ms = 0.f;
        if (cudaEventElapsedTime(&ms, ev.first, ev.second) == cudaSuccess) in->timedMs[which] += ms;
        in->timedLaunches[which]++;
        cudaEventDestroy(ev.first);
        cudaEventDestroy(ev.second);
    }
    in->timed[which].clear();
    if (outMilliseconds) *outMilliseconds = in->timedMs[which];
    if (outLaunches) *outLaunches = in->timedLaunches[which];
    return BEAGLE_SUCCESS;
}

int b200CompressSitePatterns(int resourceNumber, int taxonCount, int siteCount, const int* inStates,
                             const double* inSiteWeights, int* outSitePatternIndices, int* outPatterns,
                             double* outWeights, int* outPatternCount) {
    BeagleResourceList* rl = beagleGetResourceList();
    if (rl == nullptr || resourceNumber < 1 || resourceNumber >= rl->length) return BEAGLE_ERROR_NO_RESOURCE;
    if (taxonCount < 1 || taxonCount > 65535 || siteCount < 0 || outPatternCount == nullptr) return BEAGLE_ERROR_OUT_OF_RANGE;
    if (siteCount > 0 && (inStates == nullptr || outSitePatternIndices == nullptr || outPatterns == nullptr ||
                          outWeights == nullptr))
        return BEAGLE_ERROR_OUT_OF_RANGE;
    const int rc = compressSitePatterns(resourceNumber - 1, taxonCount, siteCount, inStates, outSitePatternIndices,
                                        outPatterns, outWeights, outPatternCount);
    if (rc != 0) return rc;
    if (inSiteWeights != nullptr) {
        for (int p = 0; p < *outPatternCount; ++p) outWeights[p] = 0.0;
        for (int s = 0; s < siteCount; ++s) outWeights[outSitePatternIndices[s]] += inSiteWeights[s];
    }
    return BEAGLE_SUCCESS;
}

BeagleBenchmarkedResourceList* beagleGetBenchmarkedResourceList(
    int tipCount, int compactBufferCount, int stateCount, int patternCount, int categoryCount, int* resourceList,
    int resourceCount, long preferenceFlags, long requirementFlags, int eigenModelCount, int partitionCount,
    int calculateDerivatives, long benchmarkFlags) {
    (void)eigenModelCount; (void)partitionCount; (void)calculateDerivatives; (void)compactBufferCount;
    static std::mutex mu;
    static std::vector<BeagleBenchmarkedResource> results;
    static BeagleBenchmarkedResourceList list;
    static const char* kImpl = "B200-CUDA-Double";
    std::lock_guard<std::mutex> lock(mu);
    BeagleResourceList* rl = beagleGetResourceList();
    if (rl == nullptr || tipCount < 2 || stateCount < 2 || patternCount < 1 || categoryCount < 1) return nullptr;
    std::vector<int> candidates;
    if (resourceList != nullptr && resourceCount > 0) {
        for (int k = 0; k < resourceCount; ++k)
            if (resourceList[k] >= 1 && resourceList[k] < rl->length &&
                std::find(candidates.begin(), candidates.end(), resourceList[k]) == candidates.end())
                candidates.push_back(resourceList[k]);
    } else {
        for (int r = 1; r < rl->length; ++r) candidates.push_back(r);
    }
    const bool rescale = (benchmarkFlags & 2L) != 0 || (benchmarkFlags & 4L) != 0;
    const int N = tipCount, n = 2 * N - 1, S = stateCount, P = patternCount, C = categoryCount;
    std::vector<int> states(P);
    std::vector<double> evec((size_t)S * S, 0.0), eval(S), ones(std::max(std::max(C, S), P), 1.0), lengths(n - 1, 0.05);
    for (int i = 0; i < S; ++i) { evec[(size_t)i * S + i] = 1.0; eval[i] = -(double)i / S; }
    for (double& f : ones) f = 1.0;
    std::vector<double> freqs(S, 1.0 / S), weights(C, 1.0 / C), rates(C, 1.0);
    std::vector<int> probIdx(n - 1), ops, scaleIdx;
    for (int k = 0; k < n - 1; ++k) probIdx[k] = k;
    for (int k = 0; k < N - 1; ++k) {
        const int dest = N + k, c1 = k == 0 ? 0 : N + k - 1, c2 = k + 1;
        const int sw = rescale ? k : BEAGLE_OP_NONE;
        const int tuple[7] = {dest, sw, BEAGLE_OP_NONE, c1, c1, c2, c2};
        ops.insert(ops.end(), tuple, tuple + 7);
        scaleIdx.push_back(k);
    }
    results.clear();
    for (int res : candidates) {
        BeagleBenchmarkedResource br{};
        br.number = res; br.name = rl->list[res].name; br.description = rl->list[res].description;
        br.supportFlags = rl->list[res].supportFlags; br.requiredFlags = rl->list[res].requiredFlags;
        br.implName = const_cast<char*>(kImpl); br.benchedFlags = 0; br.benchmarkResult = 0.0; br.performanceRatio = 0.0;
        int one[1] = {res};
        BeagleInstanceDetails det{};
        const int inst = beagleCreateInstance(N, N - 1, N, S, P, 1, n - 1, C, N + 1, one, 1, preferenceFlags,
                                              requirementFlags, &det);
        br.returnCode = inst < 0 ? inst : BEAGLE_SUCCESS;
        if (inst >= 0) {
            br.benchedFlags = det.flags;
            int rc = BEAGLE_SUCCESS;
            for (int t = 0; t < N && rc == BEAGLE_SUCCESS; ++t) {
                for (int p = 0; p < P; ++p) states[p] = (int)((1103515245u * (unsigned)(t * 7919 + p) + 12345u) >> 16) % S;
                rc = beagleSetTipStates(inst, t, states.data());
            }
            if (rc == BEAGLE_SUCCESS) rc = beagleSetPatternWeights(inst, ones.data());
            if (rc == BEAGLE_SUCCESS) rc = beagleSetEigenDecomposition(inst, 0, evec.data(), evec.data(), eval.data());
            if (rc == BEAGLE_SUCCESS) rc = beagleSetCategoryRates(inst, rates.data());
            if (rc == BEAGLE_SUCCESS) rc = beagleSetCategoryWeights(inst, 0, weights.data());
            if (rc == BEAGLE_SUCCESS) rc = beagleSetStateFrequencies(inst, 0, freqs.data());
            double best = 0.0, logL = 0.0;
            const int root = n - 1, zero = 0, cum = rescale ? N : BEAGLE_OP_NONE;
            for (int rep = 0; rep < 6 && rc == BEAGLE_SUCCESS; ++rep) {
                const auto t0 = std::chrono::steady_clock::now();
                rc = beagleUpdateTransitionMatrices(inst, 0, probIdx.data(), nullptr, nullptr, lengths.data(), n - 1);
                if (rc == BEAGLE_SUCCESS)
                    rc = beagleUpdatePartials(inst, reinterpret_cast<const BeagleOperation*>(ops.data()), N - 1, BEAGLE_OP_NONE);
                if (rc == BEAGLE_SUCCESS && rescale) {
                    rc = beagleResetScaleFactors(inst, cum);
                    if (rc == BEAGLE_SUCCESS) rc = beagleAccumulateScaleFactors(inst, scaleIdx.data(), N - 1, cum);
                }
                if (rc == BEAGLE_SUCCESS) {
                    rc = beagleCalculateRootLogLikelihoods(inst, &root, &zero, &zero, &cum, 1, &logL);
                    if (rc == BEAGLE_ERROR_FLOATING_POINT) rc = BEAGLE_SUCCESS;
                }
                const double ms = std::chrono::duration<double, std::milli>(std::chrono::steady_clock::now() - t0).count();
                if (rep >= 2 && (best == 0.0 || ms < best)) best = ms;
            }
            br.returnCode = rc;
            br.benchmarkResult = best;
            beagleFinalizeInstance(inst);
        }
        results.push_back(br);
    }
    std::stable_sort(results.begin(), results.end(), [](const BeagleBenchmarkedResource& a, const BeagleBenchmarkedResource& b) {
        const bool oa = a.returnCode == BEAGLE_SUCCESS, ob = b.returnCode == BEAGLE_SUCCESS;
        return oa != ob ? oa : (oa && a.benchmarkResult < b.benchmarkResult);
    });
    for (BeagleBenchmarkedResource& r : results)
        r.performanceRatio = (results[0].benchmarkResult > 0.0 && r.returnCode == BEAGLE_SUCCESS)
                                 ? r.benchmarkResult / results[0].benchmarkResult : 0.0;
    list.list = results.data();
    list.length = (int)results.size();
    return list.length > 0 ? &list : nullptr;
}

int b200SetShardDevices(const int* devices, int count) {
    beagleGetResourceList();
    int n = 0;
    if (cudaGetDeviceCount(&n) != cudaSuccess) { cudaGetLastError(); n = 0; }
    if (count < 1 || count > kMaxGroup || gShardResource < 0) return BEAGLE_ERROR_OUT_OF_RANGE;
    for (int k = 0; k < count; ++k) if (devices[k] < 0 || devices[k] >= n) return BEAGLE_ERROR_OUT_OF_RANGE;
    std::lock_guard<std::mutex> lock(gMutex);
// ... 43 lines not shown
```

beast-mcmc_b200/csrc/engine.h:

```cpp
#pragma once
#include <cuda_runtime.h>
#include <cstdint>
#include <mutex>
#include <vector>

namespace b200 {

struct alignas(16) DevOp {
    double* dest;
    const double* c1;
    const double* c2;
    const void* s1;
    const void* s2;
    const double* m1;
    const double* m2;
    double* scaleWrite;
    const double* scaleRead;
    double* cumScale;
    int pBegin, pEnd;
    int srcSlot1, srcSlot2;
    int dstSlot;
    int pad_;
};

struct alignas(16) Op4 {
    int dest, c1, c2, m1;
    int m2, sw, sr, cum;
    int pBegin, pEnd;
    unsigned int slots;
    int pad_;
    int pfA, pfB, pfM1, pfM2;
};

struct CherryRef { int buf, tip1, tip2; };

template <typename T> struct EdgeRefT { const T* post; const int* states; const T* pre; const double* D; double len; };
using EdgeRef = EdgeRefT<double>;

struct HostOp { int dest, sw, sr, c1, m1, c2, m2, part, cum; int kind = 0; };
struct CumGroup { int cum, pBegin, pEnd; std::vector<int> indices; };
struct CachedPlan {
    std::vector<HostOp> key;
    std::vector<CumGroup> cumGroups;
    int n = -1;
    bool byPartition = false, fourPath = false, preOrder = false;
    unsigned long epoch = 0;
    void* dBlock = nullptr;
    size_t capacity = 0, subsOffset = 0, snapOffset = 0, tipsOffset = 0;
    std::vector<CherryRef> cherries, external;
    bool readsVirtual = false;
    std::vector<int> phaseStart, phaseDepth;
    int maxWindow = 0;
    long lastUse = 0;
    long hits = 0;
    cudaGraphExec_t graphExec = nullptr;
    bool graphFailed = false;
    int graphEigen = -2;
    unsigned graphEigenGen = 0;
    int graphInvalidations = 0;
    cudaGraph_t graph = nullptr;
    std::vector<cudaGraphNode_t> graphKernelNodes;
    bool graphAllEigen = false;
    void dropGraph() {
        if (graphExec) cudaGraphExecDestroy(graphExec);
        if (graph) cudaGraphDestroy(graph);
        graphExec = nullptr; graph = nullptr; graphKernelNodes.clear(); graphAllEigen = false;
    }
};

enum TimingClass { T_PARTIALS = 0, T_MATRICES = 1, T_ROOT = 2, T_CLASSES = 3 };

constexpr int kIncMaxOps = 64, kIncMaxMats = 8;
struct IncOp { int dest, c1, c2, m1, m2, sw, sr, flags; };
struct IncMat { int prob, rateSet; double len; };
struct IncArgs {
    void* partials; size_t stride; const uint8_t* states; double* mats; double* evecs; double* scale;
    size_t matStride;
    int S, C, Ppad, P, logScalers, nOps, nMats, pad_;
    double V[16], Vi[16], eval[4];
    double weights[8], freqs[4], rate[kIncMaxMats][8];
    const double* cum; const double* patternWeights;
    double* site; double* blockSums; unsigned int* counter; double* out;
    volatile double* hostOut; volatile unsigned long long* hostFlag; unsigned long long seq;
    IncMat mat[kIncMaxMats];
    IncOp op[kIncMaxOps];
};

constexpr int kMaxGroup = 16;
struct ExchangeSlot { double value; unsigned long long seq; };
struct Exchange {
    int rank = 0, size = 1;
    unsigned long long seq = 0;
    long long timeoutCycles = 0;
    ExchangeSlot* peers[kMaxGroup] = {};
};

struct Instance {
    int id = -1, device = 0, resource = 0;
    int tipCount = 0, nPartials = 0, nCompact = 0, S = 0, P = 0, nEigen = 0, nMatrices = 0, C = 0, nScale = 0;
    int Sp = 0, Ppad = 0, nBuffers = 0, nSets = 1;
    long flags = 0;
    bool logScalers = false, complexEigen = false;
    cudaStream_t stream = nullptr;
    int smCount = 132;
    size_t maxSmemOptin = 0;

    bool single = false;
    size_t partialsElems = 0;
    size_t elemBytes() const { return single ? sizeof(float) : sizeof(double); }
    char* partialsBase = nullptr;
    int nSlots = 0, nextSlot = 0;
    std::vector<int> slotOf;
    std::vector<char*> partials;
    uint8_t* states8Base = nullptr;
    int* states32Base = nullptr;
    std::vector<uint8_t*> states8;
    std::vector<int*> states32;
    int matCP = 0;
    size_t matStride = 0;

    double* dEigen = nullptr;
    double* dMat = nullptr;
    double* dEvec = nullptr;
    std::vector<int> matEigen;
    std::vector<unsigned> matEigenGen, eigenGen;
    std::vector<char> eigenReal;
    std::vector<double> hEigen;
    int eigenWalk = 1;
    int tipMode = 2;
    int thinTipMode = 3;
    int virtualCherries = 1;
    std::vector<int> cherryTip1, cherryTip2;
    std::vector<char> cherryStored;
    double* dRecipe = nullptr;
    double* dRates = nullptr;
    std::vector<double> hRates, hWeights, hFreqs;
    double* dWeights = nullptr;
    double* dFreqs = nullptr;
    double* dScale = nullptr;
    std::vector<char> scaleIsLog;
    double* dPatternWeights = nullptr;
    int* dPatternPartitions = nullptr;
    double* dSite = nullptr;
    double* dBlockSums = nullptr;
    double* dOut = nullptr;
    unsigned int* dCounter = nullptr;
    int lookaheadPre = 1;
    int prePhases = 1;
    int useGraphs = 1;
    int lookahead = 1;
    int forward = 1;
    double* dScratch = nullptr;
    size_t scratchDoubles = 0;
    int partitionCount = 1;
    std::vector<int> partBegin, partEnd;
    std::vector<int> hostPartitions;

    char* hStage = nullptr;
    char* dStage = nullptr;
    size_t stageSize = 0, stagePos = 0;
    double* hOut = nullptr;

    int fuseSmall = 1;
    struct PendingMat { int prob, eigen, rateSet; double len; };
    std::vector<PendingMat> pendingMats;
    std::vector<HostOp> pendingOps;
    int pendingCum = -1;
    double* hMapped = nullptr;
    double* dMapped = nullptr;
    double* dIncSums = nullptr;
    unsigned int* dIncCounter = nullptr;
    unsigned long long incSeq = 0;
    long fusedLaunches = 0;

    void* shard = nullptr;
    Exchange exchange;
    ExchangeSlot* dSlots = nullptr;
    std::vector<void*> ipcOpened;
    bool exchangeOn = false;

    bool timing = false;
    std::vector<std::pair<cudaEvent_t, cudaEvent_t>> timed[T_CLASSES];
    double timedMs[T_CLASSES] = {0, 0, 0};
    long timedLaunches[T_CLASSES] = {0, 0, 0};

    size_t walkSmemConfigured = 0, genericSmemConfigured = 0, mmaSmemConfigured[8] = {0, 0, 0, 0, 0, 0, 0, 0};
    int walkBlock = 128;
    int walkVariant = 0;
    std::vector<CachedPlan> planCache;
    int planCacheSize = 4;
    long planClock = 0;
    unsigned long bufferEpoch = 0;
    int reorder = 1;
    int thinR1 = 1;
    int stackTail = 0;
    int stackDepthMax = 12;
    int walkMinBlocks = 4;
    bool walkMinBlocksSet = false;
    int mmaWarps = 4;
    int tensorR = 2;
    int genericMma = 1;
    int walkR = 4;
    int phaseTmin = 4, phaseOversub = 0, phaseSmall = 24;
    int phaseT = 0;
};

struct Sharded;
Instance* instanceById(int id);
void exchangeRelease(Instance* in);
int shardedCreate(Instance* parent, int g, const int* devices, int tipCount, int partialsBufferCount, int compactBufferCount,
                  int stateCount, int patternCount, int eigenBufferCount, int matrixBufferCount, int categoryCount,
                  int scaleBufferCount, long preferenceFlags, long requirementFlags, void* details );
void shardedDestroy(Instance* parent);

cudaError_t launchTransitionMatrices(Instance* in, const int* dProbIdx, const int* dEigenIdx,
                                     const int* dRateSet, const double* dLengths, int count);
cudaError_t launchWalk4(Instance* in, const Op4* dOps, const int4* dSubs, int nSubs, int stackDepth, int maxWindow, bool preOrder);
cudaError_t updateWalk4EGraph(cudaGraphExec_t exec, const std::vector<cudaGraphNode_t>& kernelNodes, const double* eigen);
cudaError_t launchWalk4E(Instance* in, const Op4* dOps, const int4* dSubs, int nSubs, int maxWindow, bool aligned,
                         const double* eigen, const int4* dVirtTips);
bool walk4pServes(const Instance* in, int nSubs, int maxWindow);
cudaError_t launchCherrySnapshot(Instance* in, const int4* dItems, int count);
cudaError_t launchCherryStore(Instance* in, const int4* dItems, int count);
cudaError_t launchWalkGeneric(Instance* in, const DevOp* dOps, const int4* dSubs, int nSubs, int maxWindow, bool preOrder);
size_t edgeDerivativeWorkspace(const Instance* in, int count);
cudaError_t launchEdgeDerivatives(Instance* in, const EdgeRefT<void>* dEdges, int count, const double* weights, double* outPerPattern,
                                  double* outSum, double* outSumSq, double* partial);
int compressSitePatterns(int device, int taxa, int sites, const int* hStates, int* hPatternOfSite, int* hPatterns,
                         double* hWeights, int* hPatternCount);
int crossProductBlocks(const Instance* in, int count);
cudaError_t launchCrossProducts(Instance* in, const EdgeRefT<void>* dEdges, int count, const double* rates,
                                const double* weights, double* scratch);
cudaError_t launchRoot(Instance* in, const void* root, const double* weights, const double* freqs,
                       const double* cumScale, int pBegin, int pEnd, double* dOutSlot, const Exchange* exchange = nullptr);
cudaError_t launchIncremental(Instance* in, const IncArgs& args);
cudaError_t launchCombineMatrices(Instance* in, const int* dFirst, const int* dSecond, const int* dResult, int count, bool multiply);
cudaError_t launchExchangeSum(Instance* in, const double* dVals, int n, double* dOutJoint, const Exchange* exchange);
cudaError_t launchScaleAccumulate(Instance* in, const int* dIdx, int count, double* cum, double sign,
                                  int pBegin, int pEnd);
cudaError_t launchRescalePartialsForGet(Instance* in, double* tmp, const double* cum);

}
```

beast-mcmc_b200/csrc/walk4e.cu:

```cuda
#include "engine.h"
#include "walk4.cuh"

namespace b200 {

namespace {

__device__ __forceinline__ double absBits(double v) {
    return __hiloint2double(__double2hiint(v) & 0x7fffffff, __double2loint(v));
}

template <typename T, int CP, int R, bool ALIGNED, bool FIRST, int TIP>
__device__ __forceinline__ void childTermE(const WalkArgs& A, const double (&Vi)[16], int child, int matIdx, bool fromRegisters,
                                           int cc, size_t off0, int p0, bool catValid, int pBegin, int pEnd, double (&d)[R][4],
                                           double* tab) {
    constexpr int G = 32 / CP;
    const int S = A.S;
    const bool tip = child < 0;
    if (TIP == 2 && tip) {
        const int lane = threadIdx.x & 31;
        const uint8_t* t = A.states + (size_t)(-child - 1) * A.Ppad;
        int s[R];
#pragma unroll
        for (int r = 0; r < R; ++r) {
            const int p = p0 + r * G;
            s[r] = (ALIGNED || (catValid && p >= pBegin && p < pEnd)) ? (int)__ldg(t + p) : 4;
        }
        const double* m = A.mats + (size_t)matIdx * A.matStride;
        __syncwarp();
#pragma unroll
        for (int q = lane; q < 5 * CP; q += 32) {
            const int c = q / 5, sym = q - 5 * c;
            double v[4];
            if (sym < S && sym < 4 && c < A.C) ldg256_ro(m + (sym * CP + c) * 4, v);
            else {
#pragma unroll
                for (int i = 0; i < 4; ++i) v[i] = (i < S) ? 1.0 : 0.0;
            }
            double2* dst = reinterpret_cast<double2*>(tab + q * 4);
            dst[0] = make_double2(v[0], v[1]);
            dst[1] = make_double2(v[2], v[3]);
        }
        __syncwarp();
#pragma unroll
        for (int r = 0; r < R; ++r) {
            const double2* col = reinterpret_cast<const double2*>(tab + (cc * 5 + min(s[r], 4)) * 4);
            const double2 lo = col[0], hi = col[1];
            if (FIRST) { d[r][0] = lo.x; d[r][1] = lo.y; d[r][2] = hi.x; d[r][3] = hi.y; }
            else { d[r][0] *= lo.x; d[r][1] *= lo.y; d[r][2] *= hi.x; d[r][3] *= hi.y; }
        }
        return;
    }
    if (TIP == 1 && tip) {
        const uint8_t* t = A.states + (size_t)(-child - 1) * A.Ppad;
        const double* m = A.mats + (size_t)matIdx * A.matStride + cc * 4;
#pragma unroll
        for (int r = 0; r < R; ++r) {
            const int p = p0 + r * G;
            const int s = (ALIGNED || (catValid && p >= pBegin && p < pEnd)) ? (int)__ldg(t + p) : S;
            double v[4];
            if (s < S) ldg256_ro(m + 4 * CP * s, v);
            else {
#pragma unroll
                for (int i = 0; i < 4; ++i) v[i] = (i < S) ? 1.0 : 0.0;
            }
#pragma unroll
            for (int i = 0; i < 4; ++i) d[r][i] = FIRST ? v[i] : d[r][i] * v[i];
        }
        return;
    }
    double e[4];
    ldg256_ro(A.evecs + ((size_t)matIdx * CP + cc) * 4, e);
    const uint8_t* t = A.states + (size_t)(tip ? -child - 1 : 0) * A.Ppad;
    const T* xg = static_cast<const T*>(A.partials) + (size_t)(tip ? 0 : child) * A.stride + off0;
#pragma unroll
    for (int r = 0; r < R; ++r) {
        const int p = p0 + r * G;
        const bool live = ALIGNED || (catValid && p >= pBegin && p < pEnd);
        double x[4], u[4], y[4];
        int s = 0;
        if (tip) {
            s = live ? (int)__ldg(t + p) : S;
#pragma unroll
            for (int j = 0; j < 4; ++j) x[j] = (s == j) ? 1.0 : 0.0;
        } else if (fromRegisters) {
#pragma unroll
            for (int i = 0; i < 4; ++i) x[i] = d[r][i];
        } else if (live) {
            loadCell(xg + (size_t)r * G * 4, x);
        } else {
            x[0] = x[1] = x[2] = x[3] = 0.0;
        }
#pragma unroll
        for (int k = 0; k < 4; ++k)
            u[k] = (Vi[4 * k] * x[0] + Vi[4 * k + 1] * x[1] + Vi[4 * k + 2] * x[2] + Vi[4 * k + 3] * x[3]) * e[k];
#pragma unroll
        for (int i = 0; i < 4; ++i)
            y[i] = absBits(A.V[4 * i] * u[0] + A.V[4 * i + 1] * u[1] + A.V[4 * i + 2] * u[2] + A.V[4 * i + 3] * u[3]);
        if (tip && s >= S) {
#pragma unroll
            for (int i = 0; i < 4; ++i) y[i] = (i < S) ? 1.0 : 0.0;
        }
#pragma unroll
        for (int i = 0; i < 4; ++i) d[r][i] = FIRST ? y[i] : d[r][i] * y[i];
    }
}

template <typename T, int CP, int R, bool ALIGNED, int TIP>
__device__ __forceinline__ void walk4eBody(const WalkArgs& A) {
    constexpr int G = 32 / CP;
    const int lane = threadIdx.x & 31;
    const int warp = (blockIdx.x * blockDim.x + threadIdx.x) >> 5;
    const int c = lane / G;
    const int4 range = __ldg(A.subs + blockIdx.y);
    const int p0 = range.z + warp * (G * R) + (lane % G);
    if (range.z + warp * (G * R) >= range.w) return;
    const bool catValid = c < A.C;
    const int cc = catValid ? c : 0;
    const size_t off0 = ((size_t)cc * A.Ppad + p0) * 4;
    const int last = range.y - 1;
    __shared__ __align__(16) double tipTab[TIP == 2 ? 4 * 2 * CP * 20 : 2];
    double* tab1 = tipTab + (TIP == 2 ? ((threadIdx.x >> 5) * 2) * CP * 20 : 0);
    double* tab2 = tab1 + (TIP == 2 ? CP * 20 : 0);

    double Vi[16];
#pragma unroll
    for (int q = 0; q < 16; ++q) asm volatile("mov.f64 %0, %1;" : "=d"(Vi[q]) : "d"(A.Vi[q]));
    Op4 cur = loadOp(A.ops + range.x);
    double d[R][4];
#pragma unroll
    for (int r = 0; r < R; ++r) d[r][0] = d[r][1] = d[r][2] = d[r][3] = 0.0;
    for (int k = range.x; k <= last; ++k) {
        Op4 nxt;
        if (R == 1) nxt = loadOp(A.ops + min(k + 1, last));
        else if (lane == 0) prefetchL1(A.ops + min(k + 2, last));
#pragma unroll
        for (int w = 0; w < 2; ++w) {
            const int pf = w == 0 ? cur.pfA : cur.pfB;
            if (pf == 0) continue;
            if (pf & 1) {
                const uint8_t* t = A.states + (size_t)(pf >> 1) * A.Ppad + p0;
                if ((lane % G) == 0 && c == 0) prefetchL1(t);
            } else if (catValid) {
                const T* xg = static_cast<const T*>(A.partials) + (size_t)((pf >> 1) - 1) * A.stride + off0;
#pragma unroll
                for (int r = 0; r < R; ++r)
                    if (ALIGNED || p0 + r * G < A.Ppad) prefetchL1(xg + (size_t)r * G * 4);
            }
        }
        if (lane < 2) {
            const int mi = lane == 0 ? cur.pfM1 : cur.pfM2;
            if (mi >= 0) prefetchL1(A.evecs + (size_t)mi * CP * 4);
        } else if (TIP != 0 && lane >= 8 && lane < 16) {
            const int mi = lane < 12 ? cur.pfM1 : cur.pfM2;
            if (mi >= 0) prefetchL1(A.mats + (size_t)mi * A.matStride + (lane & 3) * 4 * CP);
        }
        childTermE<T, CP, R, ALIGNED, true, TIP>(A, Vi, cur.c1, cur.m1, (cur.pad_ & 2) != 0, cc, off0, p0, catValid, cur.pBegin, cur.pEnd, d, tab1);
        childTermE<T, CP, R, ALIGNED, false, TIP>(A, Vi, cur.c2, cur.m2, false, cc, off0, p0, catValid, cur.pBegin, cur.pEnd, d, tab2);
        if (R != 1) nxt = loadOp(A.ops + min(k + 1, last));
        T* dg = static_cast<T*>(A.partials) + (size_t)cur.dest * A.stride + off0;
#pragma unroll
        for (int r = 0; r < R; ++r) {
            const int p = p0 + r * G;
            const bool active = ALIGNED ? catValid : (catValid && p >= cur.pBegin && p < cur.pEnd);
            if (cur.sw >= 0) {
                double m = active ? fmax(fmax(d[r][0], d[r][1]), fmax(d[r][2], d[r][3])) : 0.0;
#pragma unroll
                for (int sh = G; sh < 32; sh <<= 1) m = fmax(m, __shfl_xor_sync(0xffffffffu, m, sh));
                if (m == 0.0) m = 1.0;
                const double inv = 1.0 / m;
#pragma unroll
                for (int i = 0; i < 4; ++i) d[r][i] *= inv;
                if (active && c == 0) A.scale[(size_t)cur.sw * A.Ppad + p] = A.logScalers ? log(m) : m;
            } else if (cur.sr >= 0) {
                double f = active ? A.scale[(size_t)cur.sr * A.Ppad + p] : 1.0;
                if (A.logScalers) f = exp(f);
                const double inv = 1.0 / f;
#pragma unroll
                for (int i = 0; i < 4; ++i) d[r][i] *= inv;
            }
            roundCell<T>(d[r]);
            if (active) storeCell(dg + (size_t)r * G * 4, d[r]);
        }
        cur = nxt;
    }
}

template <int CP, int R, bool ALIGNED, int MINB, int TIP>
__global__ void __launch_bounds__(128, MINB)
k_walk4e(const WalkArgs A) {
    walk4eBody<double, CP, R, ALIGNED, TIP>(A);
}

template <int CP, int R, bool ALIGNED, int MINB, int TIP>
__global__ void __launch_bounds__(128, MINB)
k_walk4es(const WalkArgs A) {
    walk4eBody<float, CP, R, ALIGNED, TIP>(A);
}

__device__ __forceinline__ void cpAsync16(void* smemDst, const void* gmemSrc) {
    const unsigned sAddr = (unsigned)__cvta_generic_to_shared(smemDst);
    asm volatile("cp.async.ca.shared.global [%0], [%1], 16;" :: "r"(sAddr), "l"(gmemSrc) : "memory");
}
template <int BYTES>
__device__ __forceinline__ void cpAsyncSmall(void* smemDst, const void* gmemSrc) {
    const unsigned sAddr = (unsigned)__cvta_generic_to_shared(smemDst);
    asm volatile("cp.async.ca.shared.global [%0], [%1], %2;" :: "r"(sAddr), "l"(gmemSrc), "n"(BYTES) : "memory");
}

template <int CP, int R, bool VIRT>
struct WarpStage {
    static constexpr int G = 32 / CP, NP = G * R, TABLES = VIRT ? 4 : 2;
    double mat[TABLES][5 * CP * 4];
    double ev[2][CP * 4];
    alignas(16) unsigned char st[TABLES][NP < 16 ? 16 : NP];
};

template <typename T, int CP, int R, bool VIRT>
__device__ __forceinline__ void walk4pBody(const WalkArgs& A) {
    constexpr int G = 32 / CP, NP = G * R;
    constexpr int PIECE = NP < 16 ? NP : 16;
    static_assert(NP % PIECE == 0 && (PIECE == 4 || PIECE == 8 || PIECE == 16), "state-byte staging");
    constexpr int TABLES = WarpStage<CP, R, VIRT>::TABLES;
    constexpr int RECQ = sizeof(Op4) / 16 + (VIRT ? 1 : 0);
    __shared__ __align__(16) WarpStage<CP, R, VIRT> stages[4][2];
    __shared__ __align__(16) Op4 rings[4][4];
    __shared__ __align__(16) int4 tipRings[4][VIRT ? 4 : 1];
    int lane;
    asm volatile("mov.u32 %0, %%laneid;" : "=r"(lane));
    const int wib = threadIdx.x >> 5;
    const int warp = (blockIdx.x * blockDim.x + threadIdx.x) >> 5;
    const int c = lane / G;
    const int4 range = __ldg(A.subs + blockIdx.y);
    const int pBase = range.z + warp * NP;
    if (pBase >= range.w) return;
    const int p0 = pBase + (lane % G);
    const bool catValid = c < A.C;
    const int cc = catValid ? c : 0;
    const size_t off0 = ((size_t)cc * A.Ppad + p0) * 4;
    const int last = range.y - 1, S = A.S;
    WarpStage<CP, R, VIRT>* stage = stages[wib];
    Op4* ring = rings[wib];
    int4* tipRing = tipRings[wib];

    for (int q = lane; q < 2 * TABLES * CP * 4; q += 32) {
        const int tbl = q / (CP * 4), e = q % (CP * 4), gc = e >> 2, i = e & 3;
        stage[tbl / TABLES].mat[tbl % TABLES][(i >> 1) * 10 * CP + 2 * (4 * CP + gc) + (i & 1)] = (i < S) ? 1.0 : 0.0;
    }
    auto stageBlock = [&](double* tab, const double* src) {
#pragma unroll
        for (int q = lane; q < CP * 8; q += 32)
            cpAsync16(&tab[(q & 1) * 10 * CP + 2 * (((q >> 1) % CP) * 4 + q / (2 * CP))], src + 2 * q);
    };
    auto fetchRecord = [&](int j) {
        if (VIRT && lane == RECQ - 1) cpAsync16(&tipRing[j & 3], A.virtTips + j);
        else cpAsync16(reinterpret_cast<char*>(&ring[j & 3]) + 16 * lane, reinterpret_cast<const char*>(A.ops + j) + 16 * lane);
    };
    struct Rec { int dest, c1, c2, sw, sr, flags, pfA, pfB; };
    auto issueOperands = [&](int j) -> Rec {
        const int4 rec = *reinterpret_cast<const int4*>(&ring[j & 3]);
        const int4 rec2 = *(reinterpret_cast<const int4*>(&ring[j & 3]) + 1);
        const int flags = ring[j & 3].pad_;
        const int2 pf = *reinterpret_cast<const int2*>(&ring[j & 3].pfA);
        const int m2 = rec2.x;
        WarpStage<CP, R, VIRT>& sg = stage[j & 1];
#pragma unroll
        for (int ch = 0; ch < 2; ++ch) {
            const int child = ch == 0 ? rec.y : rec.z, m = ch == 0 ? rec.w : m2;
            const bool virt = VIRT && (flags & (4 << ch)) != 0;
            if (child < 0) {
                stageBlock(sg.mat[ch], A.mats + (size_t)m * A.matStride);
            } else {
                if (virt) {
                    const double* rcp = A.recipes + (size_t)child * 32 * CP;
                    stageBlock(sg.mat[ch], rcp);
                    stageBlock(sg.mat[TABLES - 2 + ch], rcp + 16 * CP);
                }
                if (lane < CP * 2) cpAsync16(&sg.ev[ch][2 * lane], A.evecs + (size_t)m * CP * 4 + 2 * lane);
            }
        }
        constexpr int SL = NP / PIECE;
        auto statePiece = [&](int q) {
            const int t = q / SL, piece = q % SL, ch = t & 1;
            const int child = ch == 0 ? rec.y : rec.z;
            int tip = t < 2 && child < 0 ? -child - 1 : -1;
            if (VIRT && (flags & (4 << ch)) != 0) {
                const int4 vt = tipRing[j & 3];
                tip = t == 0 ? vt.x : t == 1 ? vt.z : t == 2 ? vt.y : vt.w;
            }
            if (tip >= 0) cpAsyncSmall<PIECE>(&sg.st[t][PIECE * piece], A.states + (size_t)tip * A.Ppad + pBase + PIECE * piece);
        };
        if (lane < RECQ) {
            if (j + 1 <= last) fetchRecord(j + 1);
        } else if (lane < RECQ + TABLES * SL) {
            statePiece(lane - RECQ);
        }
        if constexpr (RECQ + TABLES * SL > 32) {
            if (lane < RECQ + TABLES * SL - 32) statePiece(lane + 32 - RECQ);
        }
        asm volatile("cp.async.commit_group;" ::: "memory");
        return Rec{rec.x, rec.y, rec.z, rec2.y, rec2.z, flags, pf.x, pf.y};
    };
    if (lane < RECQ) fetchRecord(range.x);
    asm volatile("cp.async.commit_group;" ::: "memory");
    asm volatile("cp.async.wait_group 0;" ::: "memory");
    __syncwarp();
    Rec nxt = issueOperands(range.x);
    asm volatile("cp.async.wait_group 0;" ::: "memory");
    __syncwarp();

    double Vi[16];
#pragma unroll
    for (int q = 0; q < 16; ++q) asm volatile("mov.f64 %0, %1;" : "=d"(Vi[q]) : "d"(A.Vi[q]));
    double d[R][4];
#pragma unroll
    for (int r = 0; r < R; ++r) d[r][0] = d[r][1] = d[r][2] = d[r][3] = 0.0;

    for (int k = range.x; k <= last; ++k) {
        const Rec cur = nxt;
        if (k + 1 <= last) nxt = issueOperands(k + 1);
        const WarpStage<CP, R, VIRT>& sg = stage[k & 1];
#pragma unroll
        for (int w = 0; w < 2; ++w) {
            const int pf = w == 0 ? cur.pfA : cur.pfB;
            if (pf == 0 || (pf & 1) || !catValid) continue;
            const T* xg = static_cast<const T*>(A.partials) + (size_t)((pf >> 1) - 1) * A.stride + off0;
#pragma unroll
            for (int r = 0; r < R; ++r) prefetchL1(xg + (size_t)r * G * 4);
        }
#pragma unroll
        for (int ch = 0; ch < 2; ++ch) {
            const int child = ch == 0 ? cur.c1 : cur.c2;
            if (child < 0) {
#pragma unroll
                for (int r = 0; r < R; ++r) {
                    const int sym = sg.st[ch][(lane % G) + r * G];
                    const int e2 = 2 * (sym < S ? cc * 4 + sym : 4 * CP + cc);
                    const double2 lo = *reinterpret_cast<const double2*>(&sg.mat[ch][e2]);
                    const double2 hi = *reinterpret_cast<const double2*>(&sg.mat[ch][10 * CP + e2]);
                    if (ch == 0) { d[r][0] = lo.x; d[r][1] = lo.y; d[r][2] = hi.x; d[r][3] = hi.y; }
                    else { d[r][0] *= lo.x; d[r][1] *= lo.y; d[r][2] *= hi.x; d[r][3] *= hi.y; }
                }
            } else {
                const double2* ep = reinterpret_cast<const double2*>(&sg.ev[ch][cc * 4]);
                const double2 e01 = ep[0], e23 = ep[1];
                const double e[4] = {e01.x, e01.y, e23.x, e23.y};
                const bool fromRegisters = ch == 0 && (cur.flags & 2) != 0;
                const bool virt = VIRT && (cur.flags & (4 << ch)) != 0;
                const T* xg = static_cast<const T*>(A.partials) + (size_t)child * A.stride + off0;
#pragma unroll
                for (int r = 0; r < R; ++r) {
                    double x[4], u[4], y[4];
                    if (fromRegisters) {
#pragma unroll
                        for (int i = 0; i < 4; ++i) x[i] = d[r][i];
                    } else if (virt) {
                        const int symA = sg.st[ch][(lane % G) + r * G], symB = sg.st[TABLES - 2 + ch][(lane % G) + r * G];
                        const int eA = 2 * (symA < S ? cc * 4 + symA : 4 * CP + cc);
                        const int eB = 2 * (symB < S ? cc * 4 + symB : 4 * CP + cc);
                        const double2 aLo = *reinterpret_cast<const double2*>(&sg.mat[ch][eA]);
                        const double2 aHi = *reinterpret_cast<const double2*>(&sg.mat[ch][10 * CP + eA]);
                        const double2 bLo = *reinterpret_cast<const double2*>(&sg.mat[TABLES - 2 + ch][eB]);
                        const double2 bHi = *reinterpret_cast<const double2*>(&sg.mat[TABLES - 2 + ch][10 * CP + eB]);
                        x[0] = aLo.x * bLo.x; x[1] = aLo.y * bLo.y; x[2] = aHi.x * bHi.x; x[3] = aHi.y * bHi.y;
                        roundCell<T>(x);
                    } else {
                        loadCell(xg + (size_t)r * G * 4, x);
                    }
#pragma unroll
                    for (int q = 0; q < 4; ++q)
                        u[q] = (Vi[4 * q] * x[0] + Vi[4 * q + 1] * x[1] + Vi[4 * q + 2] * x[2] + Vi[4 * q + 3] * x[3]) * e[q];
#pragma unroll
                    for (int i = 0; i < 4; ++i)
                        y[i] = absBits(A.V[4 * i] * u[0] + A.V[4 * i + 1] * u[1] + A.V[4 * i + 2] * u[2] + A.V[4 * i + 3] * u[3]);
#pragma unroll
                    for (int i = 0; i < 4; ++i) d[r][i] = ch == 0 ? y[i] : d[r][i] * y[i];
                }
            }
        }
        T* dg = static_cast<T*>(A.partials) + (size_t)cur.dest * A.stride + off0;
#pragma unroll
        for (int r = 0; r < R; ++r) {
            const int p = p0 + r * G;
            if (cur.sw >= 0) {
                double m = catValid ? fmax(fmax(d[r][0], d[r][1]), fmax(d[r][2], d[r][3])) : 0.0;
#pragma unroll
                for (int sh = G; sh < 32; sh <<= 1) m = fmax(m, __shfl_xor_sync(0xffffffffu, m, sh));
                if (m == 0.0) m = 1.0;
                const double inv = 1.0 / m;
#pragma unroll
                for (int i = 0; i < 4; ++i) d[r][i] *= inv;
                if (c == 0) A.scale[(size_t)cur.sw * A.Ppad + p] = A.logScalers ? log(m) : m;
            } else if (cur.sr >= 0) {
                double f = A.scale[(size_t)cur.sr * A.Ppad + p];
                if (A.logScalers) f = exp(f);
                const double inv = 1.0 / f;
#pragma unroll
                for (int i = 0; i < 4; ++i) d[r][i] *= inv;
            }
            roundCell<T>(d[r]);
            if (catValid) storeCell(dg + (size_t)r * G * 4, d[r]);
        }
        asm volatile("cp.async.wait_group 0;" ::: "memory");
        __syncwarp();
    }
}

template <int CP, int R, int MINB>
__global__ void __launch_bounds__(128, MINB)
k_walk4p(const WalkArgs A) {
    walk4pBody<double, CP, R, false>(A);
}

template <int CP, int R, int MINB>
__global__ void __launch_bounds__(128, MINB)
k_walk4ps(const WalkArgs A) {
    walk4pBody<float, CP, R, false>(A);
}

template <int CP, int R, int MINB>
__global__ void __launch_bounds__(128, MINB)
k_walk4pv(const WalkArgs A) {
    walk4pBody<double, CP, R, true>(A);
}

template <int CP, int R, int MINB>
__global__ void __launch_bounds__(128, MINB)
k_walk4pvs(const WalkArgs A) {
    walk4pBody<float, CP, R, true>(A);
}

template <typename T, int CP, int R, int MINB>
cudaError_t launchP(Instance* in, const WalkArgs& A, dim3 grid) {
    if constexpr (sizeof(T) == 4) k_walk4ps<CP, R, MINB><<<grid, 128, 0, in->stream>>>(A);
    else k_walk4p<CP, R, MINB><<<grid, 128, 0, in->stream>>>(A);
    return cudaGetLastError();
}

template <typename T, int CP, int R>
cudaError_t launchPV(Instance* in, const WalkArgs& A, dim3 grid) {
    if constexpr (sizeof(T) == 4) k_walk4pvs<CP, R, 3><<<grid, 128, 0, in->stream>>>(A);
    else k_walk4pv<CP, R, 3><<<grid, 128, 0, in->stream>>>(A);
    return cudaGetLastError();
}

__global__ void k_cherry_snapshot(const int4* items, const double* mats, size_t matStride, double* recipes, int blk) {
    const int4 it = items[blockIdx.x];
    for (int q = threadIdx.x; q < 2 * blk; q += blockDim.x)
        recipes[(size_t)it.x * 2 * blk + q] = mats[(size_t)(q < blk ? it.y : it.z) * matStride + q % blk];
}

template <typename T>
__device__ __forceinline__ void cherryStoreBody(const int4* items, int count, T* partials, size_t stride,
                                                const uint8_t* states, const double* recipes, int S, int C, int CP, int Ppad) {
    const int q = blockIdx.x * blockDim.x + threadIdx.x;
    if (q >= C * Ppad) return;
    const int c = q / Ppad, p = q - c * Ppad;
    for (int k = blockIdx.y; k < count; k += gridDim.y) {
        const int4 it = items[k];
        const int sA = states[(size_t)it.z * Ppad + p], sB = states[(size_t)it.w * Ppad + p];
        const double* ra = recipes + (size_t)it.y * 32 * CP;
        const double* rb = ra + 16 * CP;
        double v[4];
#pragma unroll
        for (int i = 0; i < 4; ++i) {
            const double a = sA < S ? ra[(sA * CP + c) * 4 + i] : (i < S ? 1.0 : 0.0);
            const double b = sB < S ? rb[(sB * CP + c) * 4 + i] : (i < S ? 1.0 : 0.0);
            v[i] = a * b;
        }
        roundCell<T>(v);
        storeCell(partials + (size_t)it.x * stride + (size_t)q * 4, v);
    }
}

__global__ void k_cherry_store(const int4* items, int count, double* partials, size_t stride, const uint8_t* states,
                               const double* recipes, int S, int C, int CP, int Ppad) {
    cherryStoreBody(items, count, partials, stride, states, recipes, S, C, CP, Ppad);
}

__global__ void k_cherry_store_f32(const int4* items, int count, float* partials, size_t stride, const uint8_t* states,
                                const double* recipes, int S, int C, int CP, int Ppad) {
    cherryStoreBody(items, count, partials, stride, states, recipes, S, C, CP, Ppad);
}

template <typename T, int CP, int R, bool ALIGNED, int MINB, int TIP>
cudaError_t launchK(Instance* in, const WalkArgs& A, dim3 grid) {
    if constexpr (sizeof(T) == 4) k_walk4es<CP, R, ALIGNED, MINB, TIP><<<grid, 128, 0, in->stream>>>(A);
    else k_walk4e<CP, R, ALIGNED, MINB, TIP><<<grid, 128, 0, in->stream>>>(A);
    return cudaGetLastError();
}

int phaseR(const Instance* in, int nSubs, int maxWindow) {
    const int G = 32 / in->matCP;
    const long walks = (long)nSubs * ((maxWindow + G * in->walkR - 1) / (G * in->walkR));
    if ((in->thinR1 && walks < (long)in->smCount * 8) || in->walkR == 1) return 1;
    if (in->matCP == 4 && (in->walkR == 8 || in->walkR == 2)) return in->walkR;
    return 4;
}

bool stagedWalk(const Instance* in, int R, bool aligned) {
    const int G = 32 / in->matCP;
    return aligned && in->Ppad % (G * R) == 0 && in->matCP <= 8 && G * R >= 4 && (R == 1 ? in->thinTipMode : in->tipMode) == 3;
}

template <typename T, int CP, int R>
cudaError_t launchR(Instance* in, WalkArgs& A, int nSubs, int maxWindow, bool aligned, bool virt) {
    constexpr int G = 32 / CP;
    constexpr int TIPD = CP <= 8 ? 2 : 0;
    const int warps = (maxWindow + G * R - 1) / (G * R);
    dim3 grid((warps + 3) / 4, nSubs);
    if constexpr (CP <= 8 && G * R >= 4) {
        if (stagedWalk(in, R, aligned)) {
            if (virt) {
                if constexpr (R == 8) return cudaErrorInvalidValue;
                else return launchPV<T, CP, R>(in, A, grid);
            }
            if constexpr (CP == 4) {
                const int minb = in->walkMinBlocksSet ? in->walkMinBlocks : 3;
                if (minb >= 6) return launchP<T, CP, R, 6>(in, A, grid);
                if (minb == 5) return launchP<T, CP, R, 5>(in, A, grid);
                if (minb == 3) return launchP<T, CP, R, 3>(in, A, grid);
            }
            return launchP<T, CP, R, 4>(in, A, grid);
        }
    }
    if (virt) return cudaErrorInvalidValue;
    if (!aligned || in->Ppad % (G * R) != 0) return launchK<T, CP, R, false, 4, TIPD>(in, A, grid);
    if constexpr (CP == 4 && R >= 2) {
        const int minb = in->walkMinBlocks, tip = in->tipMode;
        if (tip == 0) {
            if (minb >= 5) return launchK<T, CP, R, true, 5, 0>(in, A, grid);
            if (minb == 3) return launchK<T, CP, R, true, 3, 0>(in, A, grid);
            return launchK<T, CP, R, true, 4, 0>(in, A, grid);
        }
        if (tip == 1) {
            if (minb >= 5) return launchK<T, CP, R, true, 5, 1>(in, A, grid);
            return launchK<T, CP, R, true, 4, 1>(in, A, grid);
        }
        if (minb >= 6) return launchK<T, CP, R, true, 6, 2>(in, A, grid);
        if (minb == 5) return launchK<T, CP, R, true, 5, 2>(in, A, grid);
        if (minb == 3) return launchK<T, CP, R, true, 3, 2>(in, A, grid);
    }
    return launchK<T, CP, R, true, 4, TIPD>(in, A, grid);
}

template <typename T, int CP>
cudaError_t launchCP(Instance* in, WalkArgs& A, int nSubs, int maxWindow, bool aligned, bool virt) {
    const int R = phaseR(in, nSubs, maxWindow);
    if (R == 1) return launchR<T, CP, 1>(in, A, nSubs, maxWindow, aligned, virt);
    if constexpr (CP == 4) {
        if (R == 8) return launchR<T, CP, 8>(in, A, nSubs, maxWindow, aligned, virt);
        if (R == 2) return launchR<T, CP, 2>(in, A, nSubs, maxWindow, aligned, virt);
    }
    return launchR<T, CP, 4>(in, A, nSubs, maxWindow, aligned, virt);
}

}

bool walk4pServes(const Instance* in, int nSubs, int maxWindow) {
    if (in->matCP == 0) return false;
    const int R = phaseR(in, nSubs, maxWindow);
    return R != 8 && stagedWalk(in, R, true);
}

cudaError_t launchWalk4E(Instance* in, const Op4* dOps, const int4* dSubs, int nSubs, int maxWindow, bool aligned,
                         const double* eigen, const int4* dVirtTips) {
    const bool virt = dVirtTips != nullptr;
    if (nSubs <= 0) return cudaSuccess;
    WalkArgs A;
    A.ops = dOps; A.subs = dSubs; A.partials = in->partialsBase; A.stride = in->partialsElems;
    A.states = in->states8Base; A.mats = in->dMat; A.scale = in->dScale;
    A.S = in->S; A.C = in->C; A.Ppad = in->Ppad; A.logScalers = in->logScalers ? 1 : 0;
    A.matStride = in->matStride; A.matMmaOffset = 16 * in->matCP;
    A.evecs = in->dEvec;
    A.recipes = in->dRecipe;
    A.virtTips = dVirtTips;
    if (virt && in->dRecipe == nullptr) return cudaErrorInvalidValue;
    for (int q = 0; q < 16; ++q) { A.V[q] = eigen[q]; A.Vi[q] = eigen[16 + q]; }
    if (in->single) {
        switch (in->matCP) {
            case 1: return launchCP<float, 1>(in, A, nSubs, maxWindow, aligned, virt);
            case 2: return launchCP<float, 2>(in, A, nSubs, maxWindow, aligned, virt);
            case 8: return launchCP<float, 8>(in, A, nSubs, maxWindow, aligned, virt);
            default: return launchCP<float, 4>(in, A, nSubs, maxWindow, aligned, virt);
        }
    }
    switch (in->matCP) {
#ifndef B200_W4E_QUICK
        case 1: return launchCP<double, 1>(in, A, nSubs, maxWindow, aligned, virt);
        case 2: return launchCP<double, 2>(in, A, nSubs, maxWindow, aligned, virt);
        case 8: return launchCP<double, 8>(in, A, nSubs, maxWindow, aligned, virt);
        case 16: return launchCP<double, 16>(in, A, nSubs, maxWindow, aligned, virt);
        case 32: return launchCP<double, 32>(in, A, nSubs, maxWindow, aligned, virt);
#endif
        default: return launchCP<double, 4>(in, A, nSubs, maxWindow, aligned, virt);
    }
}

cudaError_t launchCherrySnapshot(Instance* in, const int4* dItems, int count) {
    if (count <= 0) return cudaSuccess;
    k_cherry_snapshot<<<count, 128, 0, in->stream>>>(dItems, in->dMat, in->matStride, in->dRecipe, 16 * in->matCP);
    return cudaGetLastError();
}

cudaError_t launchCherryStore(Instance* in, const int4* dItems, int count) {
    if (count <= 0) return cudaSuccess;
    const dim3 grid((in->C * in->Ppad + 255) / 256, std::min(count, 65535));
    if (in->single)
        k_cherry_store_f32<<<grid, 256, 0, in->stream>>>(dItems, count, reinterpret_cast<float*>(in->partialsBase),
                                                      in->partialsElems, in->states8Base, in->dRecipe, in->S, in->C,
                                                      in->matCP, in->Ppad);
    else
        k_cherry_store<<<grid, 256, 0, in->stream>>>(dItems, count, reinterpret_cast<double*>(in->partialsBase),
                                                     in->partialsElems, in->states8Base, in->dRecipe, in->S, in->C,
                                                     in->matCP, in->Ppad);
    return cudaGetLastError();
}

cudaError_t updateWalk4EGraph(cudaGraphExec_t exec, const std::vector<cudaGraphNode_t>& kernelNodes, const double* eigen) {
    for (cudaGraphNode_t node : kernelNodes) {
        cudaKernelNodeParams kp;
        cudaError_t e = cudaGraphKernelNodeGetParams(node, &kp);
        if (e != cudaSuccess) return e;
        if (kp.func == reinterpret_cast<void*>(k_cherry_snapshot)) continue;
        if (kp.kernelParams == nullptr || kp.kernelParams[0] == nullptr) return cudaErrorInvalidValue;
        WalkArgs A = *static_cast<const WalkArgs*>(kp.kernelParams[0]);
        for (int q = 0; q < 16; ++q) { A.V[q] = eigen[q]; A.Vi[q] = eigen[16 + q]; }
        void* args[1] = {&A};
        kp.kernelParams = args;
        kp.extra = nullptr;
        e = cudaGraphExecKernelNodeSetParams(exec, node, &kp);
        if (e != cudaSuccess) return e;
    }
    return cudaSuccess;
}

}
```

include/libhmsbeagle_b200.h:

```cpp
#ifndef LIBHMSBEAGLE_B200_H
#define LIBHMSBEAGLE_B200_H

#ifdef __cplusplus
extern "C" {
#endif

#if defined(__GNUC__)
#define BEAGLE_DLLEXPORT __attribute__((visibility("default")))
#else
#define BEAGLE_DLLEXPORT
#endif

enum BeagleReturnCodes {
    BEAGLE_SUCCESS = 0,
    BEAGLE_ERROR_GENERAL = -1,
    BEAGLE_ERROR_OUT_OF_MEMORY = -2,
    BEAGLE_ERROR_UNIDENTIFIED_EXCEPTION = -3,
    BEAGLE_ERROR_UNINITIALIZED_INSTANCE = -4,
    BEAGLE_ERROR_OUT_OF_RANGE = -5,
    BEAGLE_ERROR_NO_RESOURCE = -6,
    BEAGLE_ERROR_NO_IMPLEMENTATION = -7,
    BEAGLE_ERROR_FLOATING_POINT = -8
};

// ... 71 lines not shown
    int length;
} BeagleBenchmarkedResourceList;

typedef struct {
    int destinationPartials;
    int destinationScaleWrite;
    int destinationScaleRead;
    int child1Partials;
    int child1TransitionMatrix;
    int child2Partials;
    int child2TransitionMatrix;
} BeagleOperation;

typedef struct {
    int destinationPartials;
    int destinationScaleWrite;
    int destinationScaleRead;
    int child1Partials;
    int child1TransitionMatrix;
    int child2Partials;
    int child2TransitionMatrix;
    int partition;
    int cumulativeScaleIndex;
} BeagleOperationByPartition;

BEAGLE_DLLEXPORT const char* beagleGetVersion(void);
BEAGLE_DLLEXPORT const char* beagleGetCitation(void);
BEAGLE_DLLEXPORT BeagleResourceList* beagleGetResourceList(void);
BEAGLE_DLLEXPORT BeagleBenchmarkedResourceList* beagleGetBenchmarkedResourceList(
    int tipCount, int compactBufferCount, int stateCount, int patternCount, int categoryCount,
    int* resourceList, int resourceCount, long preferenceFlags, long requirementFlags,
    int eigenModelCount, int partitionCount, int calculateDerivatives, long benchmarkFlags);

BEAGLE_DLLEXPORT int beagleCreateInstance(int tipCount, int partialsBufferCount, int compactBufferCount,
                                          int stateCount, int patternCount, int eigenBufferCount,
                                          int matrixBufferCount, int categoryCount, int scaleBufferCount,
                                          int* resourceList, int resourceCount, long preferenceFlags,
                                          long requirementFlags, BeagleInstanceDetails* returnInfo);
BEAGLE_DLLEXPORT int beagleFinalizeInstance(int instance);
BEAGLE_DLLEXPORT int beagleFinalize(void);
BEAGLE_DLLEXPORT int beagleSetCPUThreadCount(int instance, int threadCount);

BEAGLE_DLLEXPORT int beagleSetTipStates(int instance, int tipIndex, const int* inStates);
BEAGLE_DLLEXPORT int beagleGetTipStates(int instance, int tipIndex, int* outStates);
BEAGLE_DLLEXPORT int beagleSetTipPartials(int instance, int tipIndex, const double* inPartials);
BEAGLE_DLLEXPORT int beagleSetPartials(int instance, int bufferIndex, const double* inPartials);
BEAGLE_DLLEXPORT int beagleGetPartials(int instance, int bufferIndex, int scaleIndex, double* outPartials);
BEAGLE_DLLEXPORT int beagleSetEigenDecomposition(int instance, int eigenIndex, const double* inEigenVectors,
                                                 const double* inInverseEigenVectors,
                                                 const double* inEigenValues);
BEAGLE_DLLEXPORT int beagleSetStateFrequencies(int instance, int stateFrequenciesIndex,
                                               const double* inStateFrequencies);
BEAGLE_DLLEXPORT int beagleSetCategoryWeights(int instance, int categoryWeightsIndex,
                                              const double* inCategoryWeights);
BEAGLE_DLLEXPORT int beagleSetCategoryRates(int instance, const double* inCategoryRates);
BEAGLE_DLLEXPORT int beagleSetCategoryRatesWithIndex(int instance, int categoryRatesIndex,
                                                     const double* inCategoryRates);
BEAGLE_DLLEXPORT int beagleSetPatternWeights(int instance, const double* inPatternWeights);
BEAGLE_DLLEXPORT int beagleSetPatternPartitions(int instance, int partitionCount, const int* inPatternPartitions);

BEAGLE_DLLEXPORT int beagleUpdateTransitionMatrices(int instance, int eigenIndex, const int* probabilityIndices,
                                                    const int* firstDerivativeIndices,
                                                    const int* secondDerivativeIndices,
                                                    const double* edgeLengths, int count);
BEAGLE_DLLEXPORT int beagleUpdateTransitionMatricesWithMultipleModels(
    int instance, const int* eigenIndices, const int* categoryRateIndices, const int* probabilityIndices,
    const int* firstDerivativeIndices, const int* secondDerivativeIndices, const double* edgeLengths, int count);
BEAGLE_DLLEXPORT int beagleSetTransitionMatrix(int instance, int matrixIndex, const double* inMatrix,
                                               double paddedValue);
BEAGLE_DLLEXPORT int beagleGetTransitionMatrix(int instance, int matrixIndex, double* outMatrix);
BEAGLE_DLLEXPORT int beagleSetDifferentialMatrix(int instance, int matrixIndex, const double* inMatrix);
BEAGLE_DLLEXPORT int beagleConvolveTransitionMatrices(int instance, const int* firstIndices,
                                                      const int* secondIndices, const int* resultIndices,
                                                      int matrixCount);
BEAGLE_DLLEXPORT int beagleAddTransitionMatrices(int instance, const int* firstIndices, const int* secondIndices,
                                                 const int* resultIndices, int matrixCount);
BEAGLE_DLLEXPORT int beagleTransposeTransitionMatrices(int instance, const int* inputIndices,
                                                       const int* resultIndices, int matrixCount);

BEAGLE_DLLEXPORT int beagleUpdatePartials(int instance, const BeagleOperation* operations, int operationCount,
                                          int cumulativeScaleIndex);
BEAGLE_DLLEXPORT int beagleUpdatePartialsByPartition(int instance, const BeagleOperationByPartition* operations,
                                                     int operationCount);
BEAGLE_DLLEXPORT int beagleWaitForPartials(int instance, const int* destinationPartials,
                                           int destinationPartialsCount);
BEAGLE_DLLEXPORT int beagleUpdatePrePartials(int instance, const BeagleOperation* operations, int operationCount,
                                             int cumulativeScaleIndex);
BEAGLE_DLLEXPORT int beagleUpdatePrePartialsByPartition(int instance, const BeagleOperationByPartition* operations,
                                                        int operationCount);

BEAGLE_DLLEXPORT int beagleAccumulateScaleFactors(int instance, const int* scaleIndices, int count,
                                                  int cumulativeScaleIndex);
BEAGLE_DLLEXPORT int beagleAccumulateScaleFactorsByPartition(int instance, const int* scaleIndices, int count,
                                                             int cumulativeScaleIndex, int partitionIndex);
BEAGLE_DLLEXPORT int beagleRemoveScaleFactors(int instance, const int* scaleIndices, int count,
                                              int cumulativeScaleIndex);
BEAGLE_DLLEXPORT int beagleRemoveScaleFactorsByPartition(int instance, const int* scaleIndices, int count,
                                                         int cumulativeScaleIndex, int partitionIndex);
BEAGLE_DLLEXPORT int beagleResetScaleFactors(int instance, int cumulativeScaleIndex);
BEAGLE_DLLEXPORT int beagleResetScaleFactorsByPartition(int instance, int cumulativeScaleIndex, int partitionIndex);
BEAGLE_DLLEXPORT int beagleCopyScaleFactors(int instance, int destScalingIndex, int srcScalingIndex);
BEAGLE_DLLEXPORT int beagleGetScaleFactors(int instance, int srcScalingIndex, double* outScaleFactors);
BEAGLE_DLLEXPORT int beagleGetLogScaleFactors(int instance, int srcScalingIndex, double* outLogScaleFactors);

BEAGLE_DLLEXPORT int beagleCalculateRootLogLikelihoods(int instance, const int* bufferIndices,
                                                       const int* categoryWeightsIndices,
                                                       const int* stateFrequenciesIndices,
                                                       const int* cumulativeScaleIndices, int count,
                                                       double* outSumLogLikelihood);
BEAGLE_DLLEXPORT int beagleCalculateRootLogLikelihoodsByPartition(
    int instance, const int* bufferIndices, const int* categoryWeightsIndices, const int* stateFrequenciesIndices,
    const int* cumulativeScaleIndices, const int* partitionIndices, int partitionCount, int count,
    double* outSumLogLikelihoodByPartition, double* outSumLogLikelihood);
BEAGLE_DLLEXPORT int beagleCalculateCrossProductDerivative(int instance, const int* postBufferIndices,
                                                           const int* preBufferIndices, const int* categoryRatesIndices,
                                                           const int* categoryWeightsIndices, const double* edgeLengths,
                                                           int count, double* outSumDerivatives,
                                                           double* outSumSquaredDerivatives);
BEAGLE_DLLEXPORT int beagleCalculateEdgeDerivatives(int instance, const int* postBufferIndices, const int* preBufferIndices,
                                                    const int* derivativeMatrixIndices, const int* categoryWeightsIndices,
                                                    int count, double* outDerivatives, double* outSumDerivatives,
                                                    double* outSumSquaredDerivatives);
BEAGLE_DLLEXPORT int beagleGetSiteLogLikelihoods(int instance, double* outLogLikelihoods);

BEAGLE_DLLEXPORT int b200SetKernelTiming(int instance, int enable);
BEAGLE_DLLEXPORT int b200GetKernelTiming(int instance, int which, double* outMilliseconds, long* outLaunches);
BEAGLE_DLLEXPORT const char* b200GetSourceHash(void);
BEAGLE_DLLEXPORT long b200GetFusedLaunches(int instance);
BEAGLE_DLLEXPORT void* b200HostAlloc(long bytes);
BEAGLE_DLLEXPORT void b200HostFree(void* p);
BEAGLE_DLLEXPORT int b200RootLogLikelihoodDevice(int instance, int bufferIndex, int categoryWeightsIndex,
                                                 int stateFrequenciesIndex, int cumulativeScaleIndex,
                                                 void** outDevicePointer, void** outStream);

BEAGLE_DLLEXPORT int b200SetShardDevices(const int* devices, int count);
BEAGLE_DLLEXPORT int b200ExchangeConnectLocal(const int* instances, int count);
BEAGLE_DLLEXPORT int b200ExchangeCreate(int instance, int rank, int size, void* outIpcHandle64);
BEAGLE_DLLEXPORT int b200ExchangeConnect(int instance, const void* allIpcHandles64);

BEAGLE_DLLEXPORT int b200RootLogLikelihoodsByPartitionDevice(int instance, const int* bufferIndices,
                                                             const int* categoryWeightsIndices,
                                                             const int* stateFrequenciesIndices,
                                                             const int* cumulativeScaleIndices, const int* partitionIndices,
                                                             int partitionCount, void** outDevicePointer, void** outStream);

BEAGLE_DLLEXPORT int b200CompressSitePatterns(int resourceNumber, int taxonCount, int siteCount, const int* inStates,
                                              const double* inSiteWeights, int* outSitePatternIndices, int* outPatterns,
                                              double* outWeights, int* outPatternCount);

BEAGLE_DLLEXPORT int b200DebugPlan(const int* operations, int operationCount, int bufferCount, int fixedT, int wantSubs,
                                   int minT, int smallRemainder, int preOrder, int* outOrder, int* outSubs,
                                   int* outPhaseStart, int* outCounts);

#ifdef __cplusplus
}
#endif
#endif
```

Baseline: 2355.

## Keep sibling partials in a shared-memory stack slot during staged tree walks

Adds a host-side liveness pass that assigns up to three shared-memory stack slots per subtree walk. Intermediate partials that a later op in the same subtree reads can then be taken from shared memory instead of global memory, and the prefetch encoding skips children that are served from the stack. The staged walk kernels are launched with dynamic shared memory sized to the slot depth. The aim is to cut global-memory round trips for internal node partials, at the risk of lower occupancy from the added shared memory per block.

```diff
diff --git a/beast-mcmc_b200/beagle.py b/beast-mcmc_b200/beagle.py
--- a/beast-mcmc_b200/beagle.py
+++ b/beast-mcmc_b200/beagle.py
@@ -161,6 +161,7 @@
     "b200HostAlloc": ([_L], C.c_void_p),
     "b200HostFree": ([C.c_void_p], None),
     "b200DebugPlan": ([_I if False else _IP, _I, _I, _I, _I, _I, _I, _I, _IP, _IP, _IP, _IP], _I),
+    "b200DebugStackSlots": ([_IP, _I, _I, _I, _I, _I, _I, _IP, _IP, _IP, _IP], _I),
     "b200RootLogLikelihoodDevice": ([_I, _I, _I, _I, _I, C.POINTER(C.c_void_p), C.POINTER(C.c_void_p)], _I),
 }
 
diff --git a/beast-mcmc_b200/csrc/api.cu b/beast-mcmc_b200/csrc/api.cu
--- a/beast-mcmc_b200/csrc/api.cu
+++ b/beast-mcmc_b200/csrc/api.cu
@@ -382,8 +382,74 @@
     }
 }
 
+void forwardFromPrevious(Op4& d, const Op4& pv, bool preOrder, int4* tip) {
+    if (pv.pBegin != d.pBegin || pv.pEnd != d.pEnd) return;
+    const bool v1 = (d.pad_ & 4) != 0, v2 = (d.pad_ & 8) != 0;
+    if (d.c1 >= 0 && !v1 && d.c1 == pv.dest) d.pad_ |= 2;
+    else if (!preOrder && d.c2 >= 0 && !v2 && d.c2 == pv.dest) {
+        std::swap(d.c1, d.c2); std::swap(d.m1, d.m2);
+        if (tip) *tip = make_int4(tip->z, tip->w, tip->x, tip->y);
+        d.pad_ = (d.pad_ & ~12) | (v1 ? 8 : 0) | 2;
+    }
+}
+
+void assignStackSlots(std::vector<Op4>& ops, const std::vector<Sub>& subs, int depth, std::vector<int>& subDepth,
+                      long& fromStack, long& fromMemory) {
+    auto memoryChild = [](const Op4& d, int ch) -> int {
+        const int c = ch == 0 ? d.c1 : d.c2;
+        if (c < 0 || (d.pad_ & (4 << ch)) || (ch == 0 && (d.pad_ & 2))) return -1;
+        return c;
+    };
+    int keys = 1;
+    for (const Op4& d : ops) keys = std::max(keys, 1 + std::max(d.dest, std::max(d.c1, d.c2)));
+    std::vector<int> lastRead(keys, -1), slotOf(keys, -1), freeAt(keys, -1), lastReadOf(ops.size(), -1);
+    subDepth.assign(subs.size(), 0);
+    for (size_t s = 0; s < subs.size(); ++s) {
+        const int b = subs[s].begin, e = subs[s].end;
+        for (int pos = e - 1; pos >= b; --pos) {
+            const Op4& d = ops[pos];
+            lastReadOf[pos] = lastRead[d.dest];
+            lastRead[d.dest] = -1;
+            for (int ch = 0; ch < 2; ++ch) {
+                const int c = memoryChild(d, ch);
+                if (c >= 0 && lastRead[c] < 0) lastRead[c] = pos;
+            }
+        }
+        unsigned freeMask = (1u << depth) - 1u;
+        for (int pos = b; pos < e; ++pos) {
+            Op4& d = ops[pos];
+            int src[2] = {0xFF, 0xFF};
+            for (int ch = 0; ch < 2; ++ch) {
+                const int c = memoryChild(d, ch);
+                if (c < 0) continue;
+                if (slotOf[c] >= 0) { src[ch] = slotOf[c]; ++fromStack; } else ++fromMemory;
+            }
+            for (int ch = 0; ch < 2; ++ch) {
+                const int c = memoryChild(d, ch);
+                if (c >= 0 && slotOf[c] >= 0 && freeAt[c] == pos) { freeMask |= 1u << slotOf[c]; slotOf[c] = -1; }
+            }
+            if (slotOf[d.dest] >= 0) { freeMask |= 1u << slotOf[d.dest]; slotOf[d.dest] = -1; }
+            int dst = 0xFF;
+            if (lastReadOf[pos] > pos && freeMask != 0) {
+                dst = __builtin_ctz(freeMask);
+                freeMask &= ~(1u << dst);
+                slotOf[d.dest] = dst;
+                freeAt[d.dest] = lastReadOf[pos];
+                subDepth[s] = std::max(subDepth[s], dst + 1);
+            }
+            d.slots = (unsigned)src[0] | ((unsigned)src[1] << 8) | ((unsigned)dst << 16);
+        }
+        for (int pos = b; pos < e; ++pos) {
+            const Op4& d = ops[pos];
+            lastRead[d.dest] = slotOf[d.dest] = -1;
+            for (int ch = 0; ch < 2; ++ch) if (memoryChild(d, ch) >= 0) lastRead[memoryChild(d, ch)] = -1;
+        }
+    }
+}
+
 cudaError_t launchPlan(Instance* in, const void* dOps, const void* dSubs, const std::vector<int>& phaseStart,
-                       const std::vector<int>& phaseDepth, bool fourPath, int maxWindow, bool preOrder, int eigenSlot = -1,
+                       const std::vector<int>& phaseDepth, const std::vector<int>& phaseSlots, bool fourPath, int maxWindow,
+                       bool preOrder, int eigenSlot = -1,
                        bool aligned = false, const void* dSnap = nullptr, int nSnap = 0, const void* dVirtTips = nullptr) {
     const bool virt = dVirtTips != nullptr;
     cudaError_t e = cudaSuccess;
@@ -397,7 +463,8 @@
         TimedScope ts(in, T_PARTIALS);
         if (fourPath && eigenSlot >= 0 && !preOrder && (ph >= phaseDepth.size() || phaseDepth[ph] == 0)) {
             e = launchWalk4E(in, static_cast<const Op4*>(dOps), static_cast<const int4*>(dSubs) + s0, s1 - s0, maxWindow,
-                             aligned, in->hEigen.data() + (size_t)eigenSlot * 36, static_cast<const int4*>(dVirtTips));
+                             aligned, in->hEigen.data() + (size_t)eigenSlot * 36, static_cast<const int4*>(dVirtTips),
+                             ph < phaseSlots.size() ? phaseSlots[ph] : 0);
             continue;
         }
         if (virt) return cudaErrorInvalidValue;
@@ -547,7 +614,7 @@
                 if (cp.graphExec == nullptr && !cp.graphFailed && cp.hits >= 2 && !in->timing &&
                     cudaStreamBeginCapture(in->stream, cudaStreamCaptureModeThreadLocal) == cudaSuccess) {
                     const cudaError_t e1 = launchPlan(in, cp.dBlock, static_cast<char*>(cp.dBlock) + cp.subsOffset, cp.phaseStart,
-                                                      cp.phaseDepth, cp.fourPath, cp.maxWindow, cp.preOrder, eigenSlot,
+                                                      cp.phaseDepth, cp.phaseSlots, cp.fourPath, cp.maxWindow, cp.preOrder, eigenSlot,
                                                       !cp.byPartition, dSnap, nSnap, dTips);
                     cp.graphEigen = eigenSlot;
                     cp.graphEigenGen = eigenGenNow;
@@ -588,7 +655,7 @@
                 }
             }
             CUDA_OK(launchPlan(in, cp.dBlock, static_cast<char*>(cp.dBlock) + cp.subsOffset, cp.phaseStart, cp.phaseDepth,
-                               cp.fourPath, cp.maxWindow, cp.preOrder, eigenSlot, !cp.byPartition, dSnap, nSnap,
+                               cp.phaseSlots, cp.fourPath, cp.maxWindow, cp.preOrder, eigenSlot, !cp.byPartition, dSnap, nSnap,
                                dTips));
             CUDA_OK(accumulateInList(in, cp.cumGroups));
             noteScaleWrites(in, hops);
@@ -825,17 +892,8 @@
             d.pfA = d.pfB = 0; d.pfM1 = d.pfM2 = -1;
             if (readsVirtual)
                 virtTips[pos] = make_int4(v1 ? vt1[o.c1] : 0, v1 ? vt2[o.c1] : 0, v2 ? vt1[o.c2] : 0, v2 ? vt2[o.c2] : 0);
-            if (in->forward && !(maxDepth > 0 && subStack[subOfPos[pos]]) && pos > plan.subs[subOfPos[pos]].begin) {
-                const Op4& pv = ops4[pos - 1];
-                if (pv.pBegin == d.pBegin && pv.pEnd == d.pEnd) {
-                    if (!t1 && !v1 && d.c1 == pv.dest) d.pad_ |= 2;
-                    else if (!preOrder && !t2 && !v2 && d.c2 == pv.dest) {
-                        std::swap(d.c1, d.c2); std::swap(d.m1, d.m2);
-                        if (readsVirtual) { int4& t = virtTips[pos]; t = make_int4(t.z, t.w, t.x, t.y); }
-                        d.pad_ = (d.pad_ & ~12) | (v1 ? 8 : 0) | 2;
-                    }
-                }
-            }
+            if (in->forward && !(maxDepth > 0 && subStack[subOfPos[pos]]) && pos > plan.subs[subOfPos[pos]].begin)
+                forwardFromPrevious(d, ops4[pos - 1], preOrder, readsVirtual ? &virtTips[pos] : nullptr);
         } else {
             DevOp& d = dops[pos];
             memset(&d, 0, sizeof d);
@@ -863,6 +921,14 @@
             }
         }
     }
+    std::vector<int> phaseSlots(std::max(nPhases, 1), 0);
+    long fromStack = 0, fromMemory = 0;
+    if (fourPath && eigenSlot >= 0 && !preOrder && !byPartition && maxDepth == 0 && in->stackSlots > 0 && walkStackBuilt(in)) {
+        std::vector<int> subDepth;
+        assignStackSlots(ops4, plan.subs, in->stackSlots, subDepth, fromStack, fromMemory);
+        for (int ph = 0; ph < nPhases; ++ph)
+            for (int q = plan.phaseStart[ph]; q < plan.phaseStart[ph + 1]; ++q) phaseSlots[ph] = std::max(phaseSlots[ph], subDepth[q]);
+    }
     if (fourPath && in->lookahead && (!preOrder || in->lookaheadPre)) {
         std::vector<char> thick(plan.subs.size(), 0);
         const long perSub = (maxWindow + (32 / in->matCP) * in->walkR - 1) / ((32 / in->matCP) * in->walkR);
@@ -875,13 +941,13 @@
             for (int pos = plan.subs[sIdx].begin; pos + 1 < plan.subs[sIdx].end; ++pos) {
                 Op4& d = ops4[pos];
                 const Op4& nx = ops4[pos + 1];
-                auto enc = [&](int child, bool fromRegisters, bool virt) -> int {
-                    if (fromRegisters || virt) return 0;
+                auto enc = [&](int child, bool fromRegisters, bool virt, bool fromStack) -> int {
+                    if (fromRegisters || virt || fromStack) return 0;
                     if (child < 0) return ((-child - 1) << 1) | 1;
                     return child == d.dest ? 0 : ((child + 1) << 1);
                 };
-                d.pfA = enc(nx.c1, (nx.pad_ & 2) != 0, (nx.pad_ & 4) != 0);
-                d.pfB = enc(nx.c2, false, (nx.pad_ & 8) != 0);
+                d.pfA = enc(nx.c1, (nx.pad_ & 2) != 0, (nx.pad_ & 4) != 0, (nx.slots & 0xFF) != 0xFF);
+                d.pfB = enc(nx.c2, false, (nx.pad_ & 8) != 0, ((nx.slots >> 8) & 0xFF) != 0xFF);
                 if (d.pfA == 0) { d.pfA = d.pfB; d.pfB = 0; }
                 d.pfM1 = nx.m1; d.pfM2 = nx.m2;
             }
@@ -891,7 +957,8 @@
         int fwd = 0, internal = 0;
         for (const Op4& d : ops4) { fwd += (d.pad_ & 2) != 0; internal += (d.c1 >= 0) + (d.c2 >= 0); }
         fprintf(stderr, "[b200-beagle] plan: %d ops (%zu virtual cherries), %zu subtrees, %d phases, %d internal children, "
-                "%d forwarded in registers\n", nL, cherries.size(), plan.subs.size(), nPhases, internal, fwd);
+                "%d forwarded in registers, %ld read from the stack, %ld from memory\n", nL, cherries.size(), plan.subs.size(),
+                nPhases, internal, fwd, fromStack, fromMemory);
     }
     const size_t opBytes = (fourPath ? sizeof(Op4) : sizeof(DevOp)) * (size_t)nL;
     const size_t subBytes = sizeof(Sub) * plan.subs.size();
@@ -918,7 +985,7 @@
     void* dSubs = static_cast<char*>(dOps) + subsOffset;
     std::vector<int> depths(plan.phaseStart.size(), 0);
     for (size_t ph = 0; ph + 1 < plan.phaseStart.size(); ++ph) depths[ph] = (maxDepth > 0 && ph < phaseDepth.size()) ? phaseDepth[ph] : 0;
-    cudaError_t e = launchPlan(in, dOps, dSubs, plan.phaseStart, depths, fourPath, maxWindow, preOrder, eigenSlot, !byPartition,
+    cudaError_t e = launchPlan(in, dOps, dSubs, plan.phaseStart, depths, phaseSlots, fourPath, maxWindow, preOrder, eigenSlot, !byPartition,
                                static_cast<char*>(dOps) + snapOffset, (int)snap.size(),
                                readsVirtual ? static_cast<char*>(dOps) + tipsOffset : nullptr);
     if (e == cudaSuccess) e = accumulateInList(in, cumGroups);
@@ -946,6 +1013,7 @@
             slot->subsOffset = subsOffset; slot->snapOffset = snapOffset; slot->tipsOffset = tipsOffset;
             slot->cherries = cherries; slot->external = external; slot->readsVirtual = readsVirtual;
             slot->phaseStart = plan.phaseStart; slot->phaseDepth = depths;
+            slot->phaseSlots = phaseSlots;
             slot->fourPath = fourPath; slot->maxWindow = maxWindow; slot->preOrder = preOrder;
             slot->lastUse = ++in->planClock;
             slot->cumGroups = cumGroups;
@@ -1092,6 +1160,8 @@
     in->walkVariant = envInt("B200_WALK_VARIANT", 0);
     in->reorder = envInt("B200_REORDER", 1);
     in->forward = envInt("B200_FORWARD", 1);
+    in->stackSlots = envInt("B200_WALK_STACK_SLOTS", 1) != 0 ? kStackSlots : 0;
+    in->debugLog = getenv("B200_BEAGLE_DEBUG") != nullptr;
     in->lookahead = envInt("B200_LOOKAHEAD", 1);
     in->useGraphs = envInt("B200_GRAPHS", 1);
     in->prePhases = envInt("B200_PRE_PHASES", 1);
@@ -2160,6 +2230,48 @@
     return BEAGLE_SUCCESS;
 }
 
+int b200DebugStackSlots(const int* operations, int operationCount, int bufferCount, int tipCount, int wantSubs, int minT,
+                        int smallRemainder, int* outRecords, int* outSubs, int* outPhaseStart, int* outCounts) {
+    if (operationCount <= 0 || bufferCount <= 0 || tipCount < 0 || tipCount > bufferCount) return BEAGLE_ERROR_OUT_OF_RANGE;
+    std::vector<HostOp> hops(operationCount);
+    for (int k = 0; k < operationCount; ++k) {
+        const int* o = operations + 7 * k;
+        for (int f : {o[0], o[3], o[5]}) if (f < 0 || f >= bufferCount) return BEAGLE_ERROR_OUT_OF_RANGE;
+        hops[k] = {o[0], o[1], o[2], o[3], o[4], o[5], o[6], 0, -1};
+    }
+    Plan plan;
+    planPhases(hops, bufferCount, true, 0, std::max(1, wantSubs), std::max(1, minT), smallRemainder, plan);
+    std::vector<Op4> ops(operationCount);
+    for (int pos = 0; pos < operationCount; ++pos) {
+        const HostOp& o = hops[plan.order[pos]];
+        Op4& d = ops[pos];
+        memset(&d, 0, sizeof d);
+        d.dest = o.dest;
+        d.c1 = o.c1 < tipCount ? -(o.c1 + 1) : o.c1;
+        d.c2 = o.c2 < tipCount ? -(o.c2 + 1) : o.c2;
+        d.m1 = o.m1; d.m2 = o.m2; d.pEnd = 1;
+        d.slots = 0xFFFFFFu;
+    }
+    for (size_t s = 0; s < plan.subs.size(); ++s)
+        for (int pos = plan.subs[s].begin + 1; pos < plan.subs[s].end; ++pos) forwardFromPrevious(ops[pos], ops[pos - 1], false, nullptr);
+    std::vector<int> subDepth;
+    long fromStack = 0, fromMemory = 0;
+    assignStackSlots(ops, plan.subs, kStackSlots, subDepth, fromStack, fromMemory);
+    for (int pos = 0; pos < operationCount; ++pos) {
+        const Op4& d = ops[pos];
+        int* r = outRecords + 5 * pos;
+        r[0] = d.dest; r[1] = d.c1; r[2] = d.c2; r[3] = d.pad_; r[4] = (int)d.slots;
+    }
+    for (size_t q = 0; q < plan.subs.size(); ++q) { outSubs[2 * q] = plan.subs[q].begin; outSubs[2 * q + 1] = plan.subs[q].end; }
+    for (size_t q = 0; q < plan.phaseStart.size(); ++q) outPhaseStart[q] = plan.phaseStart[q];
+    outCounts[0] = (int)plan.subs.size();
+    outCounts[1] = (int)plan.phaseStart.size() - 1;
+    outCounts[2] = (int)fromStack;
+    outCounts[3] = (int)fromMemory;
+    outCounts[4] = *std::max_element(subDepth.begin(), subDepth.end());
+    return BEAGLE_SUCCESS;
+}
+
 int b200SetKernelTiming(int instance, int enable) {
     SH(instance, shBroadcast(sh, [&](int c) { return b200SetKernelTiming(c, enable); }));
     GET_INSTANCE(in, instance);
diff --git a/beast-mcmc_b200/csrc/engine.h b/beast-mcmc_b200/csrc/engine.h
--- a/beast-mcmc_b200/csrc/engine.h
+++ b/beast-mcmc_b200/csrc/engine.h
@@ -49,7 +49,7 @@
     size_t capacity = 0, subsOffset = 0, snapOffset = 0, tipsOffset = 0;
     std::vector<CherryRef> cherries, external;
     bool readsVirtual = false;
-    std::vector<int> phaseStart, phaseDepth;
+    std::vector<int> phaseStart, phaseDepth, phaseSlots;
     int maxWindow = 0;
     long lastUse = 0;
     long hits = 0;
@@ -94,6 +94,8 @@
     long long timeoutCycles = 0;
     ExchangeSlot* peers[kMaxGroup] = {};
 };
+
+constexpr int kStackSlots = 3;
 
 struct Instance {
     int id = -1, device = 0, resource = 0;
@@ -150,6 +152,8 @@
     int useGraphs = 1;
     int lookahead = 1;
     int forward = 1;
+    int stackSlots = kStackSlots;
+    bool debugLog = false;
     double* dScratch = nullptr;
     size_t scratchDoubles = 0;
     int partitionCount = 1;
@@ -218,8 +222,9 @@
 cudaError_t launchWalk4(Instance* in, const Op4* dOps, const int4* dSubs, int nSubs, int stackDepth, int maxWindow, bool preOrder);
 cudaError_t updateWalk4EGraph(cudaGraphExec_t exec, const std::vector<cudaGraphNode_t>& kernelNodes, const double* eigen);
 cudaError_t launchWalk4E(Instance* in, const Op4* dOps, const int4* dSubs, int nSubs, int maxWindow, bool aligned,
-                         const double* eigen, const int4* dVirtTips);
+                         const double* eigen, const int4* dVirtTips, int stackSlots);
 bool walk4pServes(const Instance* in, int nSubs, int maxWindow);
+bool walkStackBuilt(const Instance* in);
 cudaError_t launchCherrySnapshot(Instance* in, const int4* dItems, int count);
 cudaError_t launchCherryStore(Instance* in, const int4* dItems, int count);
 cudaError_t launchWalkGeneric(Instance* in, const DevOp* dOps, const int4* dSubs, int nSubs, int maxWindow, bool preOrder);
diff --git a/beast-mcmc_b200/csrc/walk4e.cu b/beast-mcmc_b200/csrc/walk4e.cu
--- a/beast-mcmc_b200/csrc/walk4e.cu
+++ b/beast-mcmc_b200/csrc/walk4e.cu
@@ -1,3 +1,6 @@
+#include <atomic>
+#include <cstdio>
+
 #include "engine.h"
 #include "walk4.cuh"
 
@@ -207,6 +210,20 @@
     asm volatile("cp.async.ca.shared.global [%0], [%1], %2;" :: "r"(sAddr), "l"(gmemSrc), "n"(BYTES) : "memory");
 }
 
+__device__ __forceinline__ void lds256(const double2* p, double (&v)[4]) {
+    const unsigned a = (unsigned)__cvta_generic_to_shared(p);
+    asm volatile("ld.shared.v2.f64 {%0,%1}, [%4];\n\tld.shared.v2.f64 {%2,%3}, [%4+512];"
+                 : "=d"(v[0]), "=d"(v[1]), "=d"(v[2]), "=d"(v[3]) : "r"(a) : "memory");
+}
+__device__ __forceinline__ void sts256(double2* p, const double (&v)[4]) {
+    const unsigned a = (unsigned)__cvta_generic_to_shared(p);
+    asm volatile("st.shared.v2.f64 [%0], {%1,%2};\n\tst.shared.v2.f64 [%0+512], {%3,%4};"
+                 :: "r"(a), "d"(v[0]), "d"(v[1]), "d"(v[2]), "d"(v[3]) : "memory");
+}
+
+constexpr size_t stackBytes(int slots, int R) { return (size_t)slots * 4 * R * 64 * sizeof(double2); }
+__host__ __device__ constexpr bool stackBuilt(int CP, int R, int MINB) { return CP == 4 && MINB == 3 && R <= 4; }
+
 template <int CP, int R, bool VIRT>
 struct WarpStage {
     static constexpr int G = 32 / CP, NP = G * R, TABLES = VIRT ? 4 : 2;
@@ -215,7 +232,7 @@
     alignas(16) unsigned char st[TABLES][NP < 16 ? 16 : NP];
 };
 
-template <typename T, int CP, int R, bool VIRT>
+template <typename T, int CP, int R, bool VIRT, bool STACK>
 __device__ __forceinline__ void walk4pBody(const WalkArgs& A) {
     constexpr int G = 32 / CP, NP = G * R;
     constexpr int PIECE = NP < 16 ? NP : 16;
@@ -225,6 +242,7 @@
     __shared__ __align__(16) WarpStage<CP, R, VIRT> stages[4][2];
     __shared__ __align__(16) Op4 rings[4][4];
     __shared__ __align__(16) int4 tipRings[4][VIRT ? 4 : 1];
+    extern __shared__ double2 sibStack[];
     int lane;
     asm volatile("mov.u32 %0, %%laneid;" : "=r"(lane));
     const int wib = threadIdx.x >> 5;
@@ -241,6 +259,7 @@
     WarpStage<CP, R, VIRT>* stage = stages[wib];
     Op4* ring = rings[wib];
     int4* tipRing = tipRings[wib];
+    double2* const myStack = sibStack + wib * R * 64 + lane;
 
     for (int q = lane; q < 2 * TABLES * CP * 4; q += 32) {
         const int tbl = q / (CP * 4), e = q % (CP * 4), gc = e >> 2, i = e & 3;
@@ -255,11 +274,12 @@
         if (VIRT && lane == RECQ - 1) cpAsync16(&tipRing[j & 3], A.virtTips + j);
         else cpAsync16(reinterpret_cast<char*>(&ring[j & 3]) + 16 * lane, reinterpret_cast<const char*>(A.ops + j) + 16 * lane);
     };
-    struct Rec { int dest, c1, c2, sw, sr, flags, pfA, pfB; };
+    struct Rec { int dest, c1, c2, sw, sr, flags, pfA, pfB, slots; };
     auto issueOperands = [&](int j) -> Rec {
         const int4 rec = *reinterpret_cast<const int4*>(&ring[j & 3]);
         const int4 rec2 = *(reinterpret_cast<const int4*>(&ring[j & 3]) + 1);
         const int flags = ring[j & 3].pad_;
+        const int slots = STACK ? (int)ring[j & 3].slots : 0xFFFFFF;
         const int2 pf = *reinterpret_cast<const int2*>(&ring[j & 3].pfA);
         const int m2 = rec2.x;
         WarpStage<CP, R, VIRT>& sg = stage[j & 1];
@@ -298,7 +318,7 @@
             if (lane < RECQ + TABLES * SL - 32) statePiece(lane + 32 - RECQ);
         }
         asm volatile("cp.async.commit_group;" ::: "memory");
-        return Rec{rec.x, rec.y, rec.z, rec2.y, rec2.z, flags, pf.x, pf.y};
+        return Rec{rec.x, rec.y, rec.z, rec2.y, rec2.z, flags, pf.x, pf.y, slots};
     };
     if (lane < RECQ) fetchRecord(range.x);
     asm volatile("cp.async.commit_group;" ::: "memory");
@@ -346,6 +366,7 @@
                 const double e[4] = {e01.x, e01.y, e23.x, e23.y};
                 const bool fromRegisters = ch == 0 && (cur.flags & 2) != 0;
                 const bool virt = VIRT && (cur.flags & (4 << ch)) != 0;
+                const int src = STACK ? (cur.slots >> (8 * ch)) & 0xFF : 0xFF;
                 const T* xg = static_cast<const T*>(A.partials) + (size_t)child * A.stride + off0;
 #pragma unroll
                 for (int r = 0; r < R; ++r) {
@@ -363,6 +384,8 @@
                         const double2 bHi = *reinterpret_cast<const double2*>(&sg.mat[TABLES - 2 + ch][10 * CP + eB]);
                         x[0] = aLo.x * bLo.x; x[1] = aLo.y * bLo.y; x[2] = aHi.x * bHi.x; x[3] = aHi.y * bHi.y;
                         roundCell<T>(x);
+                    } else if (STACK && src != 0xFF) {
+                        lds256(myStack + (src * 4 * R + r) * 64, x);
                     } else {
                         loadCell(xg + (size_t)r * G * 4, x);
                     }
@@ -378,6 +401,7 @@
             }
         }
         T* dg = static_cast<T*>(A.partials) + (size_t)cur.dest * A.stride + off0;
+        const int dst = STACK ? (cur.slots >> 16) & 0xFF : 0xFF;
 #pragma unroll
         for (int r = 0; r < R; ++r) {
             const int p = p0 + r * G;
@@ -399,6 +423,7 @@
             }
             roundCell<T>(d[r]);
             if (catValid) storeCell(dg + (size_t)r * G * 4, d[r]);
+            if (STACK && dst != 0xFF) sts256(myStack + (dst * 4 * R + r) * 64, d[r]);
         }
         asm volatile("cp.async.wait_group 0;" ::: "memory");
         __syncwarp();
@@ -408,39 +433,60 @@
 template <int CP, int R, int MINB>
 __global__ void __launch_bounds__(128, MINB)
 k_walk4p(const WalkArgs A) {
-    walk4pBody<double, CP, R, false>(A);
+    walk4pBody<double, CP, R, false, stackBuilt(CP, R, MINB)>(A);
 }
 
 template <int CP, int R, int MINB>
 __global__ void __launch_bounds__(128, MINB)
 k_walk4ps(const WalkArgs A) {
-    walk4pBody<float, CP, R, false>(A);
+    walk4pBody<float, CP, R, false, stackBuilt(CP, R, MINB)>(A);
 }
 
 template <int CP, int R, int MINB>
 __global__ void __launch_bounds__(128, MINB)
 k_walk4pv(const WalkArgs A) {
-    walk4pBody<double, CP, R, true>(A);
+    walk4pBody<double, CP, R, true, stackBuilt(CP, R, MINB)>(A);
 }
 
 template <int CP, int R, int MINB>
 __global__ void __launch_bounds__(128, MINB)
 k_walk4pvs(const WalkArgs A) {
-    walk4pBody<float, CP, R, true>(A);
+    walk4pBody<float, CP, R, true, stackBuilt(CP, R, MINB)>(A);
+}
+
+template <auto KERNEL, int CP, int R, int MINB>
+cudaError_t launchStaged(Instance* in, const WalkArgs& A, dim3 grid, int stackSlots) {
+    const size_t smem = stackBuilt(CP, R, MINB) ? stackBytes(stackSlots, R) : 0;
+    if (smem > 0) {
+        static std::atomic<unsigned long long> limitSet{0};
+        const unsigned long long bit = 1ull << (in->device & 63);
+        if (!(limitSet.load() & bit)) {
+            cudaError_t e = cudaFuncSetAttribute(KERNEL, cudaFuncAttributeMaxDynamicSharedMemorySize,
+                                                 (int)stackBytes(kStackSlots, R));
+            if (e != cudaSuccess) return e;
+            limitSet.fetch_or(bit);
+        }
+    }
+    if (in->debugLog) {
+        const auto kernel = KERNEL;
+        int blocks = 0;
+        cudaOccupancyMaxActiveBlocksPerMultiprocessor(&blocks, kernel, 128, smem);
+        fprintf(stderr, "[b200-beagle] staged walk: %zu B sibling stack per block, %d blocks per SM\n", smem, blocks);
+    }
+    KERNEL<<<grid, 128, smem, in->stream>>>(A);
+    return cudaGetLastError();
 }
 
 template <typename T, int CP, int R, int MINB>
-cudaError_t launchP(Instance* in, const WalkArgs& A, dim3 grid) {
-    if constexpr (sizeof(T) == 4) k_walk4ps<CP, R, MINB><<<grid, 128, 0, in->stream>>>(A);
-    else k_walk4p<CP, R, MINB><<<grid, 128, 0, in->stream>>>(A);
-    return cudaGetLastError();
+cudaError_t launchP(Instance* in, const WalkArgs& A, dim3 grid, int stackSlots) {
+    if constexpr (sizeof(T) == 4) return launchStaged<k_walk4ps<CP, R, MINB>, CP, R, MINB>(in, A, grid, stackSlots);
+    else return launchStaged<k_walk4p<CP, R, MINB>, CP, R, MINB>(in, A, grid, stackSlots);
 }
 
 template <typename T, int CP, int R>
-cudaError_t launchPV(Instance* in, const WalkArgs& A, dim3 grid) {
-    if constexpr (sizeof(T) == 4) k_walk4pvs<CP, R, 3><<<grid, 128, 0, in->stream>>>(A);
-    else k_walk4pv<CP, R, 3><<<grid, 128, 0, in->stream>>>(A);
-    return cudaGetLastError();
+cudaError_t launchPV(Instance* in, const WalkArgs& A, dim3 grid, int stackSlots) {
+    if constexpr (sizeof(T) == 4) return launchStaged<k_walk4pvs<CP, R, 3>, CP, R, 3>(in, A, grid, stackSlots);
+    else return launchStaged<k_walk4pv<CP, R, 3>, CP, R, 3>(in, A, grid, stackSlots);
 }
 
 __global__ void k_cherry_snapshot(const int4* items, const double* mats, size_t matStride, double* recipes, int blk) {
@@ -503,7 +549,7 @@
 }
 
 template <typename T, int CP, int R>
-cudaError_t launchR(Instance* in, WalkArgs& A, int nSubs, int maxWindow, bool aligned, bool virt) {
+cudaError_t launchR(Instance* in, WalkArgs& A, int nSubs, int maxWindow, bool aligned, bool virt, int stackSlots) {
     constexpr int G = 32 / CP;
     constexpr int TIPD = CP <= 8 ? 2 : 0;
     const int warps = (maxWindow + G * R - 1) / (G * R);
@@ -512,15 +558,15 @@
         if (stagedWalk(in, R, aligned)) {
             if (virt) {
                 if constexpr (R == 8) return cudaErrorInvalidValue;
-                else return launchPV<T, CP, R>(in, A, grid);
+                else return launchPV<T, CP, R>(in, A, grid, stackSlots);
             }
             if constexpr (CP == 4) {
                 const int minb = in->walkMinBlocksSet ? in->walkMinBlocks : 3;
-                if (minb >= 6) return launchP<T, CP, R, 6>(in, A, grid);
-                if (minb == 5) return launchP<T, CP, R, 5>(in, A, grid);
-                if (minb == 3) return launchP<T, CP, R, 3>(in, A, grid);
-            }
-            return launchP<T, CP, R, 4>(in, A, grid);
+                if (minb >= 6) return launchP<T, CP, R, 6>(in, A, grid, stackSlots);
+                if (minb == 5) return launchP<T, CP, R, 5>(in, A, grid, stackSlots);
+                if (minb == 3) return launchP<T, CP, R, 3>(in, A, grid, stackSlots);
+            }
+            return launchP<T, CP, R, 4>(in, A, grid, stackSlots);
         }
     }
     if (virt) return cudaErrorInvalidValue;
@@ -544,16 +590,21 @@
 }
 
 template <typename T, int CP>
-cudaError_t launchCP(Instance* in, WalkArgs& A, int nSubs, int maxWindow, bool aligned, bool virt) {
+cudaError_t launchCP(Instance* in, WalkArgs& A, int nSubs, int maxWindow, bool aligned, bool virt, int stackSlots) {
     const int R = phaseR(in, nSubs, maxWindow);
-    if (R == 1) return launchR<T, CP, 1>(in, A, nSubs, maxWindow, aligned, virt);
+    if (R == 1) return launchR<T, CP, 1>(in, A, nSubs, maxWindow, aligned, virt, stackSlots);
     if constexpr (CP == 4) {
-        if (R == 8) return launchR<T, CP, 8>(in, A, nSubs, maxWindow, aligned, virt);
-        if (R == 2) return launchR<T, CP, 2>(in, A, nSubs, maxWindow, aligned, virt);
-    }
-    return launchR<T, CP, 4>(in, A, nSubs, maxWindow, aligned, virt);
-}
-
+        if (R == 8) return launchR<T, CP, 8>(in, A, nSubs, maxWindow, aligned, virt, stackSlots);
+        if (R == 2) return launchR<T, CP, 2>(in, A, nSubs, maxWindow, aligned, virt, stackSlots);
+    }
+    return launchR<T, CP, 4>(in, A, nSubs, maxWindow, aligned, virt, stackSlots);
+}
+
+}
+
+bool walkStackBuilt(const Instance* in) {
+    const int minb = in->walkMinBlocksSet ? in->walkMinBlocks : 3;
+    return stackBuilt(in->matCP, in->walkR == 8 ? 8 : 4, minb);
 }
 
 bool walk4pServes(const Instance* in, int nSubs, int maxWindow) {
@@ -563,7 +614,7 @@
 }
 
 cudaError_t launchWalk4E(Instance* in, const Op4* dOps, const int4* dSubs, int nSubs, int maxWindow, bool aligned,
-                         const double* eigen, const int4* dVirtTips) {
+                         const double* eigen, const int4* dVirtTips, int stackSlots) {
     const bool virt = dVirtTips != nullptr;
     if (nSubs <= 0) return cudaSuccess;
     WalkArgs A;
@@ -578,21 +629,21 @@
     for (int q = 0; q < 16; ++q) { A.V[q] = eigen[q]; A.Vi[q] = eigen[16 + q]; }
     if (in->single) {
         switch (in->matCP) {
-            case 1: return launchCP<float, 1>(in, A, nSubs, maxWindow, aligned, virt);
-            case 2: return launchCP<float, 2>(in, A, nSubs, maxWindow, aligned, virt);
-            case 8: return launchCP<float, 8>(in, A, nSubs, maxWindow, aligned, virt);
-            default: return launchCP<float, 4>(in, A, nSubs, maxWindow, aligned, virt);
+            case 1: return launchCP<float, 1>(in, A, nSubs, maxWindow, aligned, virt, stackSlots);
+            case 2: return launchCP<float, 2>(in, A, nSubs, maxWindow, aligned, virt, stackSlots);
+            case 8: return launchCP<float, 8>(in, A, nSubs, maxWindow, aligned, virt, stackSlots);
+            default: return launchCP<float, 4>(in, A, nSubs, maxWindow, aligned, virt, stackSlots);
         }
     }
     switch (in->matCP) {
 #ifndef B200_W4E_QUICK
-        case 1: return launchCP<double, 1>(in, A, nSubs, maxWindow, aligned, virt);
-        case 2: return launchCP<double, 2>(in, A, nSubs, maxWindow, aligned, virt);
-        case 8: return launchCP<double, 8>(in, A, nSubs, maxWindow, aligned, virt);
-        case 16: return launchCP<double, 16>(in, A, nSubs, maxWindow, aligned, virt);
-        case 32: return launchCP<double, 32>(in, A, nSubs, maxWindow, aligned, virt);
+        case 1: return launchCP<double, 1>(in, A, nSubs, maxWindow, aligned, virt, stackSlots);
+        case 2: return launchCP<double, 2>(in, A, nSubs, maxWindow, aligned, virt, stackSlots);
+        case 8: return launchCP<double, 8>(in, A, nSubs, maxWindow, aligned, virt, stackSlots);
+        case 16: return launchCP<double, 16>(in, A, nSubs, maxWindow, aligned, virt, stackSlots);
+        case 32: return launchCP<double, 32>(in, A, nSubs, maxWindow, aligned, virt, stackSlots);
 #endif
-        default: return launchCP<double, 4>(in, A, nSubs, maxWindow, aligned, virt);
+        default: return launchCP<double, 4>(in, A, nSubs, maxWindow, aligned, virt, stackSlots);
     }
 }
 
diff --git a/include/libhmsbeagle_b200.h b/include/libhmsbeagle_b200.h
--- a/include/libhmsbeagle_b200.h
+++ b/include/libhmsbeagle_b200.h
@@ -247,6 +247,10 @@
                                    int minT, int smallRemainder, int preOrder, int* outOrder, int* outSubs,
                                    int* outPhaseStart, int* outCounts);
 
+BEAGLE_DLLEXPORT int b200DebugStackSlots(const int* operations, int operationCount, int bufferCount, int tipCount,
+                                         int wantSubs, int minT, int smallRemainder, int* outRecords, int* outSubs,
+                                         int* outPhaseStart, int* outCounts);
+
 #ifdef __cplusplus
 }
 #endif
```

Result: faster. 2568 (median of 6 runs) (+9.0%).
